# QuentinHuan/ENSEM3A_OpenCLRaytracer

Measured on AMD Instinct MI355X. Metric: Msamples/s Cornell box 1024x1024 64spp; 1/2/4/8-GPU scaling; HBM %peak, higher is better.
Workload: dtype f32; 1 GPU; cornell_1024_s64; scene=cornell, width=1024, height=1024, spp=64, max_bounce=4, traversal=fast, bvh=sah, parallelism=row-interleaved x1

## Files before the change

ensem3a_openclraytracer_amd/_native.py:

```python
from __future__ import annotations

import ctypes
import os
import threading

import numpy as np

from ._build import LIB

_lock = threading.Lock()
_lib = None
_host = None

RT_TRAVERSAL_FAST = 0
RT_TRAVERSAL_REF = 1
RT_BVH_REFERENCE = 0
RT_BVH_SAH = 1
RT_ERR_ARG = 1
RT_ERR_STATE = 3
RT_ACCUM_MAX_SAMPLES = 1 << 24

EXPORTED = (
    "rt_create", "rt_destroy", "rt_last_error", "rt_set_scene", "rt_set_env", "rt_set_option",
    "rt_render", "rt_render_device", "rt_tile_rows", "rt_count_work", "rt_count_work_detail", "rt_work_bytes", "rt_gamma",
    "rt_render_rgb8", "rt_rgb8_device", "rt_rgb8",
    "rt_accum_begin", "rt_accum_add", "rt_accum_add_rgb8", "rt_accum_read", "rt_accum_samples", "rt_accum_end",
    "rt_accum_begin_device", "rt_accum_add_device",
    "rt_accum_mark", "rt_accum_select", "rt_accum_select_mask", "rt_accum_select_all", "rt_accum_selection",
    "rt_accum_sample_map", "rt_accum_add_selected", "rt_accum_mark_device", "rt_accum_select_device",
    "rt_accum_select_mask_device", "rt_accum_select_all_device", "rt_accum_add_selected_device",
    "rt_accum_guides", "rt_accum_guides_device", "rt_denoise_device", "rt_accum_denoise",
    "rt_trace", "rt_trace_device",
    "rt_bvh_build", "rt_device_count", "rt_debug_math", "rt_debug_fn", "rt_debug_trace", "rt_debug_trace_clustered", "rt_debug_scene_info", "rt_debug_pixel_log",
    "rt_debug_wave_counts", "rt_debug_quantise_axis", "rt_debug_timings", "rt_debug_brute_layout",
    "rt_debug_brute_clusters", "rt_debug_brute_shell", "rt_debug_brute_near", "rt_debug_brute_quad",
    "rt_debug_brute_slices",
    "rt_debug_last_slices",
    "rt_debug_brute_refill", "rt_debug_last_refill", "rt_debug_last_launch",
    "rt_obj_parse", "rt_obj_size", "rt_obj_copy", "rt_obj_free", "rt_obj_last_error",
    "rt_scene_check", "rt_scene_last_error",
)
HOST_ONLY = ("rt_bvh_build", "rt_obj_parse", "rt_obj_size", "rt_obj_copy", "rt_obj_free", "rt_obj_last_error",
             "rt_scene_check", "rt_scene_last_error", "rt_debug_quantise_axis", "rt_debug_brute_layout",
             "rt_debug_brute_clusters", "rt_debug_brute_shell", "rt_debug_brute_near", "rt_debug_brute_quad")

_c_p = ctypes.c_void_p
_i64 = ctypes.c_int64
_i32 = ctypes.c_int


class DenoiseParams(ctypes.Structure):
    _fields_ = [("passes", ctypes.c_int), ("normal_squarings", ctypes.c_int),
                ("sigma_c", ctypes.c_float), ("sigma_p", ctypes.c_float)]

    def __init__(self, passes: int = 5, normal_squarings: int = 5, sigma_c: float = 1.5, sigma_p: float = 0.02):
        super().__init__(int(passes), int(normal_squarings), float(sigma_c), float(sigma_p))


GUIDE_FLOATS = 12

HIT_DTYPE = np.dtype([("k", np.float32), ("tri", np.int32), ("u", np.float32), ("v", np.float32)])
RAY_FLOATS = 8
RT_QUERY_CLOSEST = 0
RT_QUERY_ANY = 1
QUERY_HORIZON = 1000.0


def pack_rays(origins, directions, tmax=None) -> np.ndarray:
    o = np.asarray(origins, dtype=np.float32).reshape(-1, 3)
    d = np.asarray(directions, dtype=np.float32).reshape(-1, 3)
    if len(o) != len(d):
        raise ValueError(f"{len(o)} origins but {len(d)} directions")
    rays = np.zeros((len(o), RAY_FLOATS), np.float32)
    rays[:, 0:3] = d
    rays[:, 3:6] = o
    rays[:, 6] = QUERY_HORIZON if tmax is None else np.asarray(tmax, dtype=np.float32)
    return rays


class NativeError(RuntimeError):

    def __init__(self, status: int, message: str):
        super().__init__(f"[rt status {status}] {message}")
        self.status = status


def _preload_hip_runtime() -> None:
    import importlib.util
    try:
        spec = importlib.util.find_spec("torch")
    except (ImportError, ValueError):
        spec = None
    for d in (spec.submodule_search_locations or []) if spec else []:
        p = os.path.join(d, "lib", "libamdhip64.so")
        if os.path.exists(p):
            ctypes.CDLL(p, mode=ctypes.RTLD_GLOBAL)
            return


def lib():
    global _lib
    if _lib is not None:
        return _lib
    with _lock:
        if _lib is not None:
            return _lib
        _preload_hip_runtime()
        lib_path = os.environ.get("ENSEM3A_RT_LIB", LIB)
        if not os.path.exists(lib_path):
            raise RuntimeError(
                f"native library {lib_path} is missing: build it with "
                "`python -m ensem3a_openclraytracer_amd._build` (there is no CPU fallback)")
        L = ctypes.CDLL(lib_path)
        sig = {
            "rt_create": (_i32, [_i32, _c_p, ctypes.POINTER(_c_p)]),
            "rt_destroy": (None, [_c_p]),
            "rt_last_error": (ctypes.c_char_p, [_c_p]),
            "rt_set_scene": (_i32, [_c_p, _c_p, _i64, _c_p, _i64, _c_p, _i64, _c_p, _i64, _c_p, _i64, _c_p, _i64]),
# ... 342 lines not shown
        out = np.zeros((max(n, 1), GUIDE_FLOATS), np.float32)
        self._check(lib().rt_accum_guides(self.handle, out.ctypes.data))
        return out[:n]

    def accum_guides_device(self, d_guides_ptr: int, stream_ptr: int = 0, device_index: int = 0) -> None:
        self._check(lib().rt_accum_guides_device(self.handle, int(device_index),
                                                 _c_p(int(d_guides_ptr)) if d_guides_ptr else None,
                                                 self._stream(stream_ptr)))

    def denoise_device(self, d_rgb_ptr: int, d_guides_ptr: int, npix: int, width: int, d_out_ptr: int,
                       params: "DenoiseParams" = None, stream_ptr: int = 0, device_index: int = 0) -> None:
        self._check(lib().rt_denoise_device(self.handle, int(device_index),
                                            _c_p(int(d_rgb_ptr)) if d_rgb_ptr else None,
                                            _c_p(int(d_guides_ptr)) if d_guides_ptr else None, int(npix), int(width),
                                            ctypes.byref(params) if params is not None else None,
                                            _c_p(int(d_out_ptr)) if d_out_ptr else None, self._stream(stream_ptr)))

    def accum_denoise(self, params: "DenoiseParams" = None, out: np.ndarray = None) -> np.ndarray:
        out = self._accum_out(out, np.float32)
        self._check(lib().rt_accum_denoise(self.handle, ctypes.byref(params) if params is not None else None,
                                           out.ctypes.data))
        return out

    def trace(self, rays8, mode: int = RT_QUERY_CLOSEST) -> np.ndarray:
        r = f32(rays8)
        if r.size % RAY_FLOATS:
            raise ValueError("rays must hold 8 floats each: dir.xyz, origin.xyz, tmax, reserved")
        n = r.size // RAY_FLOATS
        out = np.zeros(n, HIT_DTYPE)
        self._check(lib().rt_trace(self.handle, ptr(r), n, int(mode), out.ctypes.data if n else None))
        return out

    def trace_device(self, device_index: int, rays_ptr: int, n: int, mode: int, out_ptr: int,
                     stream_ptr: int = 0) -> None:
        self._check(lib().rt_trace_device(self.handle, int(device_index), _c_p(int(rays_ptr)) if rays_ptr else None,
                                          int(n), int(mode), _c_p(int(out_ptr)) if out_ptr else None,
                                          self._stream(stream_ptr)))

    def rgb8(self, src, gamma: bool = False, out=None) -> np.ndarray:
        s = f32(src).reshape(-1)
        if out is None:
            out = np.zeros(s.size, dtype=np.uint8)
        self._check(lib().rt_rgb8(self.handle, ptr(s), out.ctypes.data, s.size, int(bool(gamma))))
        return out

    def rgb8_device(self, d_in_ptr: int, d_out_ptr: int, n: int, gamma: bool = False, stream_ptr: int = 0,
                    device_index: int = 0) -> None:
        self._check(lib().rt_rgb8_device(self.handle, int(device_index), _c_p(int(d_in_ptr)), _c_p(int(d_out_ptr)),
                                         int(n), int(bool(gamma)), _c_p(int(stream_ptr)) if stream_ptr else None))

    def debug_math(self, fn: int, x, y=None):
        x = f32(x)
        yy = f32(y) if y is not None else None
        out = np.zeros_like(x)
        self._check(lib().rt_debug_math(self.handle, int(fn), ptr(x), ptr(yy), out.ctypes.data, x.size))
        return out

    DEBUG_FN = {"camera": (0, 11, 3), "sun": (1, 5, 3), "hemi": (2, 6, 24), "ggx": (3, 13, 3), "ibl": (4, 4, 6),
                "mt_ref": (5, 24, 2), "mt_fast": (6, 24, 2), "box_ref": (7, 12, 1), "box_fast": (8, 13, 3)}

    def debug_fn(self, name: str, items) -> np.ndarray:
        fn, wi, wo = self.DEBUG_FN[name]
        x = f32(items)
        if x.ndim != 2 or x.shape[1] != wi:
            raise ValueError(f"{name}: items must be [n, {wi}] floats")
        out = np.zeros((x.shape[0], wo), dtype=np.float32)
        if x.shape[0]:
            self._check(lib().rt_debug_fn(self.handle, fn, ptr(x), out.ctypes.data, x.shape[0]))
        return out

    def debug_trace(self, rays, traversal: int):
        r = f32(rays).reshape(-1)
        out = np.zeros(2 * (r.size // 6), dtype=np.float32)
        self._check(lib().rt_debug_trace(self.handle, int(traversal), ptr(r), out.ctypes.data, r.size // 6))
        return out.reshape(-1, 2)

    def debug_trace_clustered(self, rays6):
        r = f32(rays6).reshape(-1, 6)
        out = np.zeros((len(r), 2), dtype=np.float32)
        info = np.zeros(4, dtype=np.int32)
        self._check(lib().rt_debug_trace_clustered(self.handle, r.ctypes.data, out.ctypes.data, len(r), info.ctypes.data))
        return out[:, 0].copy(), out[:, 1].copy().view(np.int32), info

    def debug_pixel_log(self, traversal, cam, env, npix, spp, max_bounce, pixel, cap=4096):
        c, e = f32(cam), f32(env)
        log = np.zeros((cap, 16), np.float32)
        n = ctypes.c_int(0)
        out3 = np.zeros(3, np.float32)
        self._check(lib().rt_debug_pixel_log(self.handle, int(traversal), ptr(c), ptr(e), int(npix), int(spp),
                                             int(max_bounce), int(pixel), log.ctypes.data, cap, ctypes.byref(n),
                                             out3.ctypes.data))
        return log[: n.value].copy(), out3

    def wave_counts(self, cam, env, npix, spp, max_bounce):
        c, e = f32(cam), f32(env)
        out = np.zeros(9, dtype=np.uint64)
        self._check(lib().rt_debug_wave_counts(self.handle, ptr(c), ptr(e), int(npix), int(spp), int(max_bounce),
                                               out.ctypes.data))
        keys = ("node_fetches", "tri_tests", "rays", "env_lookups", "stack_drops", "wave_trav_iters",
                "wave_render_iters", "cycles_shade", "cycles_trav")
        return {k: int(v) for k, v in zip(keys, out)}

    def scene_info(self):
        out = np.zeros(8, dtype=np.int64)
        self._check(lib().rt_debug_scene_info(self.handle, out.ctypes.data))
        return dict(fast_ok=bool(out[0]), depth=int(out[1]), nodes=int(out[2]), tris=int(out[3]),
                    brute_records=int(out[4]), brute_boxes=int(out[5]), wdq_omax=int(out[6]) * 1e-6)

    def timings(self) -> dict:
        out = np.zeros(4, dtype=np.float64)
        self._check(lib().rt_debug_timings(self.handle, out.ctypes.data))
        return dict(pack_ms=float(out[0]), upload_ms=float(out[1]), env_ms=float(out[2]), render_ms=float(out[3]))


def parse_obj(text):
    data = text.encode() if isinstance(text, str) else bytes(text)
    h = _c_p()
    H = host_lib()
    if H.rt_obj_parse(data, len(data), ctypes.byref(h)) != 0:
        raise ValueError("OBJ parse failed: " + H.rt_obj_last_error().decode(errors="replace"))
    try:
        n = [int(H.rt_obj_size(h, k)) for k in range(5)]
        vp, vn, vuv = (np.zeros(n[k], np.float32) for k in range(3))
        face = np.zeros(n[3], np.int32)
        H.rt_obj_copy(h, vp.ctypes.data, vn.ctypes.data, vuv.ctypes.data, face.ctypes.data)
    finally:
        H.rt_obj_free(h)
    return vp, vn, vuv, face, n[4]


def scene_check(V_p, V_n, faceData, materialData, bvh, layout: int = RT_BVH_SAH) -> dict:
    vp, vn, face, mat, b = f32(V_p), f32(V_n), i32(faceData), f32(materialData), f32(bvh)
    info = np.zeros(8, np.int64)
    H = host_lib()
    st = H.rt_scene_check(ptr(vp), vp.size, ptr(vn), vn.size, ptr(face), face.size, ptr(mat), mat.size,
                          ptr(b), b.size, int(layout), info.ctypes.data)
    msg = H.rt_scene_last_error().decode(errors="replace")
    if st != 0:
        raise NativeError(st, msg)
    return dict(tris=int(info[0]), nodes=int(info[1]), depth=int(info[2]), wnodes=int(info[3]),
                wdepth=int(info[4]), brute_records=int(info[5]), brute_boxes=int(info[6]), fast_ok=bool(info[7]),
                note=msg)


def brute_layout(V_p, V_n, faceData, materialData, bvh, layout: int = RT_BVH_SAH):
    vp, vn, face, mat, b = f32(V_p), f32(V_n), i32(faceData), f32(materialData), f32(bvh)
    H = host_lib()
    info = np.zeros(3, np.int64)
    args = (ptr(vp), vp.size, ptr(vn), vn.size, ptr(face), face.size, ptr(mat), mat.size, ptr(b), b.size, int(layout))
    st = H.rt_debug_brute_layout(*args, None, 0, info.ctypes.data)
    if st != 0:
        raise NativeError(st, H.rt_scene_last_error().decode(errors="replace"))
    boxes = np.zeros(int(info[2]), np.float32)
    st = H.rt_debug_brute_layout(*args, boxes.ctypes.data, boxes.size, info.ctypes.data)
    if st != 0:
        raise NativeError(st, H.rt_scene_last_error().decode(errors="replace"))
    return boxes.reshape(-1, 8), int(info[0]), int(info[1])


def brute_clusters(V_p, V_n, faceData, materialData, bvh, cluster: int = -1, layout: int = RT_BVH_SAH):
    vp, vn, face, mat, b = f32(V_p), f32(V_n), i32(faceData), f32(materialData), f32(bvh)
    H = host_lib()
    info = np.zeros(4, np.int64)
    args = (ptr(vp), vp.size, ptr(vn), vn.size, ptr(face), face.size, ptr(mat), mat.size, ptr(b), b.size, int(layout),
            int(cluster))
    st = H.rt_debug_brute_clusters(*args, None, 0, None, 0, info.ctypes.data)
    if st != 0:
        raise NativeError(st, H.rt_scene_last_error().decode(errors="replace"))
    slots, rows = np.zeros(int(info[2]), np.float32), np.zeros(int(info[3]), np.float32)
    st = H.rt_debug_brute_clusters(*args, slots.ctypes.data, slots.size, rows.ctypes.data, rows.size, info.ctypes.data)
    if st != 0:
        raise NativeError(st, H.rt_scene_last_error().decode(errors="replace"))
    return slots.reshape(-1, 8), rows.reshape(-1, 8), int(info[1])


SHELL_REC_FLOATS = 76


def brute_shell(V_p, V_n, faceData, materialData, bvh, cluster: int = -1, shell: int = -1, layout: int = RT_BVH_SAH):
    vp, vn, face, mat, b = f32(V_p), f32(V_n), i32(faceData), f32(materialData), f32(bvh)
    H = host_lib()
    info = np.zeros(3, np.int64)
    args = (ptr(vp), vp.size, ptr(vn), vn.size, ptr(face), face.size, ptr(mat), mat.size, ptr(b), b.size, int(layout),
            int(cluster), int(shell))
    st = H.rt_debug_brute_shell(*args, None, 0, info.ctypes.data)
    if st != 0:
        raise NativeError(st, H.rt_scene_last_error().decode(errors="replace"))
    if int(info[0]) == 0:
        return None
    rec = np.zeros(int(info[2]), np.float32)
    st = H.rt_debug_brute_shell(*args, rec.ctypes.data, rec.size, info.ctypes.data)
    if st != 0:
        raise NativeError(st, H.rt_scene_last_error().decode(errors="replace"))
    ints = rec[:SHELL_REC_FLOATS].view(np.int32)
    return dict(box=rec[:6].copy(), nrest=int(ints[6]), nfaces=int(ints[7]) & 0xff, faces=ints[8:20].reshape(6, 2).copy(),
                rest=rec[SHELL_REC_FLOATS:].reshape(-1, 8).copy())


NEAR_FLOOR = np.float32(0.0001) * (np.float32(1.0) - np.float32(2.0 ** -12))


def brute_near(V_p, V_n, faceData, materialData, bvh, cluster: int = -1, shell: int = -1, layout: int = RT_BVH_SAH):
    vp, vn, face, mat, b = f32(V_p), f32(V_n), i32(faceData), f32(materialData), f32(bvh)
    H = host_lib()
    info = np.zeros(2, np.int64)
    floor = np.zeros(1, np.float32)
    args = (ptr(vp), vp.size, ptr(vn), vn.size, ptr(face), face.size, ptr(mat), mat.size, ptr(b), b.size, int(layout),
            int(cluster), int(shell))
    st = H.rt_debug_brute_near(*args, None, 0, floor.ctypes.data, info.ctypes.data)
    if st != 0:
        raise NativeError(st, H.rt_scene_last_error().decode(errors="replace"))
    flags = np.zeros(int(info[0]), np.int32)
    st = H.rt_debug_brute_near(*args, flags.ctypes.data if flags.size else None, flags.size, floor.ctypes.data,
                               info.ctypes.data)
    if st != 0:
        raise NativeError(st, H.rt_scene_last_error().decode(errors="replace"))
    return flags.astype(bool), np.float32(floor[0]), int(info[1])


QUAD_BAND, QUAD_GRAZE, QUAD_DIR_MAX = np.float32(2.0 ** -8), np.float32(2.0 ** -6), np.float32(2.0)


def brute_quad(V_p, V_n, faceData, materialData, bvh, cluster: int = -1, shell: int = -1, quad: int = -1,
               layout: int = RT_BVH_SAH):
    vp, vn, face, mat, b = f32(V_p), f32(V_n), i32(faceData), f32(materialData), f32(bvh)
    flags, lines, words = np.zeros(6, np.int32), np.zeros(24, np.float32), np.zeros(18, np.int32)
    recs, guard, info = np.zeros(108, np.float32), np.zeros(3, np.float32), np.zeros(2, np.int64)
    st = host_lib().rt_debug_brute_quad(ptr(vp), vp.size, ptr(vn), vn.size, ptr(face), face.size, ptr(mat), mat.size,
                                        ptr(b), b.size, int(layout), int(cluster), int(shell), int(quad),
                                        flags.ctypes.data, lines.ctypes.data, words.ctypes.data, recs.ctypes.data,
                                        guard.ctypes.data,
                                        info.ctypes.data)
    if st != 0:
        raise NativeError(st, host_lib().rt_scene_last_error().decode(errors="replace"))
    return dict(split=(flags & 1).astype(bool), side=((flags >> 1) & 1).astype(bool), lines=lines.reshape(6, 4),
                words=words.view(np.uint32).reshape(6, 3), recs=recs.reshape(6, 2, 3, 3), guard=guard, nfaces=int(info[0]), nsplit=int(info[1]))


def brute_slices(nloc: int, lanes: int, spp: int, option: int = -1, accum_base: int = -1):
    out = np.zeros(3, np.int32)
    st = lib().rt_debug_brute_slices(int(nloc), int(lanes), int(spp), int(option), int(accum_base), out.ctypes.data)
    if st != 0:
        raise NativeError(st, "rt_debug_brute_slices: bad arguments")
    return bool(out[0]), int(out[1]), int(out[2])


def last_slices() -> int:
    return int(lib().rt_debug_last_slices())


def brute_refill(nloc: int, lanes: int, option: int = -1) -> int:
    out = np.zeros(1, np.int32)
    st = lib().rt_debug_brute_refill(int(nloc), int(lanes), int(option), out.ctypes.data)
    if st != 0:
        raise NativeError(st, "rt_debug_brute_refill: bad arguments")
    return int(out[0])


def last_refill():
    out = np.zeros(3, np.int64)
    st = lib().rt_debug_last_refill(out.ctypes.data)
    if st != 0:
        raise NativeError(st, "rt_debug_last_refill: bad arguments")
    return int(out[0]), int(out[1]), int(out[2])


LAUNCH_FIELDS = ("trav", "count", "log", "smem", "ovf", "resume", "step", "wide", "brute", "ts", "acc",
                 "team", "walk_team", "slices", "refill", "grid", "lds", "shell", "near", "quad")
BRUTE_SLICED = 4
BRUTE_REFILL = 8


def last_launch() -> dict:
    out = np.zeros(len(LAUNCH_FIELDS), np.int32)
    st = lib().rt_debug_last_launch(out.ctypes.data)
    if st != 0:
        raise NativeError(st, "rt_debug_last_launch: bad arguments")
    return {name: int(v) for name, v in zip(LAUNCH_FIELDS, out)}


def tile_rows(npix: int, width: int, row0: int, row_step: int) -> int:
    return int(lib().rt_tile_rows(int(npix), int(width), int(row0), int(row_step)))
```

ensem3a_openclraytracer_amd/csrc/rt_api.hip:

```cpp
#include <hip/hip_runtime.h>

#include <cmath>
#include <cstdarg>
#include <cstdio>
#include <algorithm>
#include <array>
#include <atomic>
#include <chrono>
#include <cstring>
#include <map>
#include <string>
#include <thread>
#include <vector>

#include "../../include/rt_api.h"
#include "../../include/rt_debug.h"
#include "rt_internal.h"
#include "scene_pack.h"

constexpr int kResumeMinBvh2 = 36, kResumeMinWide = 48;
constexpr int kDenoiseLds = 1;

using rt::HostScene;

namespace {

thread_local std::string g_thread_error;

struct DevBuf {
    void* p = nullptr;
    size_t bytes = 0;
    DevBuf() = default;
    DevBuf(const DevBuf&) = delete;
    DevBuf& operator=(const DevBuf&) = delete;
    DevBuf(DevBuf&& o) noexcept : p(o.p), bytes(o.bytes) { o.p = nullptr, o.bytes = 0; }
    DevBuf& operator=(DevBuf&& o) noexcept {
        std::swap(p, o.p);
        std::swap(bytes, o.bytes);
        return *this;
    }
    ~DevBuf() { release(); }
    void release() {
        if (p) (void)hipFree(p);
        p = nullptr;
        bytes = 0;
    }
};

struct Device {
    int id = 0;
    hipStream_t stream = nullptr;
    int cus = 0;
    DevBuf stack_ovf;
    DevBuf nodes, wnodes, wleaves, tri_fast, brute, brute_box, brute_cbox, brute_crow, bvh9, tri_geo, tri_shade, tri_frame, mat, ibl, ibl_sum, out, out8, counts, work, scratch_a, scratch_b;
    DevBuf pilot;
    DevBuf spec;
    DevBuf slice;
    DevBuf accum;
    bool acc_open = false;
    bool acc_valid = false;
    float acc_cam[10] = {0}, acc_env[5] = {0};
    int64_t acc_npix = 0, acc_nloc = 0, acc_samples = 0;
    int acc_max_bounce = 0, acc_row0 = 0, acc_row_step = 1;
    DevBuf mark, sel, all;
    bool acc_marked = false, acc_selected = false, acc_all_ready = false;
    bool acc_uniform = true;
    bool sel_all = false;
    int64_t sel_known = -1;
    int64_t acc_full = 0;
    DevBuf dn, dn_const, guides, dn_rgb, dn_guides, dn_out;
    DevBuf q_counter, q_rays, q_out;
    char* host_stage = nullptr;
    int* host_pick = nullptr;
    size_t host_stage_bytes = 0;
    hipEvent_t done = nullptr;
    hipStream_t last = nullptr;
    bool pending = false;

    Device() = default;
    Device(const Device&) = delete;
    Device& operator=(const Device&) = delete;
    ~Device() {
        (void)hipSetDevice(id);
        if (host_stage) (void)hipHostFree(host_stage);
        if (host_pick) (void)hipHostFree(host_pick);
        if (stream) (void)hipStreamDestroy(stream);
        if (done) (void)hipEventDestroy(done);
    }
};

}

struct rt_ctx {
    std::vector<Device> devs;
    HostScene hs;
    bool have_scene = false;
    bool have_env = false;
    int ibl_w = 0, ibl_h = 0;
    int traversal = RT_TRAVERSAL_FAST;
    int bvh_layout = RT_BVH_SAH;
    int brute_max = RT_BRUTE_MAX_DEFAULT;
    int brute_cluster = -1;
    int brute_shell = -1;
    int brute_near = -1;
    int brute_quad = -1;
    int resume_min = -1;
    int team = 0;
    int walk_team = 0;
    int max_waves = 0;
    int step = 0;
    int sun_skip = 1;
    int sun_any = 1;
    int block = 128;
    int bvh_width = 0;
    int fixed_point = 1;
    int sun_cache = 1;
    int pilot = -1;
    int pilot_chunk = 0;
    int pilot_levels = 0;
    int stack_lds = 0;
    int ref_stack = 20;
    int spec = -1;
    int wdq = 1;
    int handout = -1;
    int slices = -1;
    int brute_refill = -1;
    int denoise_lds = -1;
    int query_engine = 0;
    int query_grid = 0;
    bool accum_host = false;
    double t_pack_ms = 0, t_upload_ms = 0, t_env_ms = 0, t_render_ms = 0;
    std::string err;
};

namespace {

int set_err(rt_ctx* ctx, int code, const char* fmt, ...) {
    char buf[1024];
    va_list ap;
    va_start(ap, fmt);
    vsnprintf(buf, sizeof buf, fmt, ap);
    va_end(ap);
    if (ctx) ctx->err = buf;
    g_thread_error = buf;
    return code;
}

#define HIP_OR_RET(ctx, call)                                                                           \
    do {                                                                                                \
        hipError_t e_ = (call);                                                                         \
        if (e_ != hipSuccess)                                                                           \
            return set_err((ctx), RT_ERR_HIP, "%s failed: %s", #call, hipGetErrorString(e_));           \
    } while (0)

hipError_t grow(Device& d, DevBuf& b, size_t bytes) {
    bytes = std::max<size_t>(bytes, 16);
    if (b.p && b.bytes >= bytes) return hipSuccess;
    hipError_t e = d.pending ? hipEventSynchronize(d.done) : hipSuccess;
    if (e != hipSuccess) return e;
    if (b.p && (e = hipFree(b.p)) != hipSuccess) return e;
    b.p = nullptr;
    b.bytes = 0;
    if ((e = hipMalloc(&b.p, bytes)) == hipSuccess) b.bytes = bytes;
    return e;
}

hipError_t grow_stage(Device& d, size_t bytes) {
    if (d.host_stage_bytes >= bytes) return hipSuccess;
    hipError_t e = d.host_stage ? hipHostFree(d.host_stage) : hipSuccess;
    if (e != hipSuccess) return e;
    d.host_stage = nullptr;
    d.host_stage_bytes = 0;
    if ((e = hipHostMalloc((void**)&d.host_stage, bytes, hipHostMallocDefault)) == hipSuccess) d.host_stage_bytes = bytes;
    return e;
}

}

namespace {

constexpr int kStackLdsMin = 8;
hipError_t ensure_stack_ovf(Device& d, const HostScene& hs) {
    const int64_t extra = (int64_t)std::max(hs.depth, hs.wdepth) - kStackLdsMin;
    if (extra <= 0) return hipSuccess;
    return grow(d, d.stack_ovf, (size_t)std::max(d.cus, 1) * rt::kMaxLanesPerCu * (size_t)extra * sizeof(int2));
}

// ... 7 lines not shown
    d.pending = true;
    return hipEventRecord(d.done, s);
}

template <typename T>
hipError_t upload(Device& d, DevBuf& b, const std::vector<T>& v) {
    const size_t bytes = v.size() * sizeof(T);
    hipError_t e = grow(d, b, bytes);
    if (e != hipSuccess || bytes == 0) return e;
    return hipMemcpyAsync(b.p, v.data(), bytes, hipMemcpyHostToDevice, d.stream);
}

hipError_t upload_cbox(Device& d, const HostScene& hs) {
    if (hs.brute_shell.empty()) return upload(d, d.brute_cbox, hs.brute_cbox);
    std::vector<float> v(hs.brute_cbox);
    v.insert(v.end(), hs.brute_shell.begin(), hs.brute_shell.end());
    const hipError_t e = upload(d, d.brute_cbox, v);
    return e != hipSuccess ? e : hipStreamSynchronize(d.stream);
}

int upload_fast(rt_ctx* ctx, Device& d, const HostScene& hs) {
    HIP_OR_RET(ctx, hipSetDevice(d.id));
    HIP_OR_RET(ctx, order_after_last(d, d.stream));
    HIP_OR_RET(ctx, upload(d, d.nodes, hs.nodes));
    HIP_OR_RET(ctx, upload(d, d.wnodes, hs.wnodes));
    HIP_OR_RET(ctx, upload(d, d.wleaves, hs.wleaves));
    HIP_OR_RET(ctx, upload(d, d.brute, hs.brute));
    HIP_OR_RET(ctx, upload(d, d.brute_box, hs.brute_box));
    HIP_OR_RET(ctx, upload_cbox(d, hs));
    HIP_OR_RET(ctx, upload(d, d.brute_crow, hs.brute_crow));
    HIP_OR_RET(ctx, upload(d, d.tri_geo, hs.tri_geo));
    HIP_OR_RET(ctx, upload(d, d.tri_fast, hs.tri_fast));
    HIP_OR_RET(ctx, ensure_stack_ovf(d, hs));
    return RT_OK;
}

int effective_traversal(const rt_ctx* ctx) {
    return (ctx->traversal == RT_TRAVERSAL_FAST && ctx->hs.fast_ok) ? RT_TRAVERSAL_FAST : RT_TRAVERSAL_REF;
}

bool use_wide(const rt_ctx* ctx) {
    if (ctx->hs.wnodes.empty() || ctx->bvh_width == 2) return false;
    return ctx->bvh_width == 4 || (size_t)ctx->hs.nnodes * 16 * rt::kNodeF4 > rt::kWideMinBytes;
}

int resume_min_of(const rt_ctx* ctx) {
    return ctx->resume_min >= 0 ? ctx->resume_min : use_wide(ctx) ? kResumeMinWide : kResumeMinBvh2;
}

rt::DevScene dev_scene(const rt_ctx* ctx, const Device& d) {
    rt::DevScene s{};
    s.nodes = (const float4*)d.nodes.p;
    s.nnodes = ctx->hs.nnodes;
    s.root_ref = ctx->hs.root_ref;
    const bool wide = use_wide(ctx);
    s.wnodes = wide ? (const float4*)d.wnodes.p : nullptr;
    s.wleaves = wide ? (const float4*)d.wleaves.p : nullptr;
    s.wroot_ref = ctx->hs.wroot_ref;
    s.wdq_omax = wide ? ctx->hs.wdq_omax : 0.0f;
    for (int k = 0; k < 6; ++k) s.root_box[k] = ctx->hs.root_box[k];
    s.bvh9 = (const float*)d.bvh9.p;
    s.nbvh9 = ctx->hs.nbvh9;
    s.ref_stack = ctx->ref_stack;
    s.tri_geo = (const float4*)d.tri_geo.p;
    s.tri_fast = (const float4*)d.tri_fast.p;
    s.tri_shade = (const float4*)d.tri_shade.p;
    s.tri_frame = (const float4*)d.tri_frame.p;
    s.ntri = ctx->hs.ntri;
    s.mat = (const float*)d.mat.p;
    s.nmat = ctx->hs.nmat;
    s.ibl_sum = (const uint32_t*)d.ibl_sum.p;
    s.ibl_w = ctx->ibl_w;
    s.ibl_h = ctx->ibl_h;
    s.depth = wide ? std::max(ctx->hs.depth, ctx->hs.wdepth) : ctx->hs.depth;
    s.brute = (const float4*)d.brute.p;
    s.brute_box = (const float4*)d.brute_box.p;
    s.nbrute = ctx->hs.nbrute;
    s.nbox = ctx->hs.nbox;
    s.brute_cbox = (const float4*)d.brute_cbox.p;
    s.brute_crow = (const float4*)d.brute_crow.p;
    s.ncluster = ctx->hs.ncluster;
    s.ncslot = (int32_t)(ctx->hs.brute_cbox.size() / 8);
    s.nsingle4 = s.ncslot - rt::kClusterSlots * s.ncluster;
    s.host_flags = (ctx->brute_cluster < 0 ? rt::kHostClusterAuto : 0) | (ctx->hs.nquad > 0 ? rt::kHostQuad : 0);
    s.nsingle = ctx->hs.nsingle;
    s.shell = ctx->hs.nshell > 0 ? 2 * s.ncslot : 0;
    s.near_floor = s.shell && ctx->brute_near != 0 ? ctx->hs.shell_floor : 0.0f;
    s.near_mask_lo = s.near_floor != 0.0f ? (uint32_t)ctx->hs.shell_mask : 0u;
    s.near_mask_hi = s.near_floor != 0.0f ? (uint32_t)(ctx->hs.shell_mask >> 32) : 0u;
    s.stack_lds = std::min<int32_t>(s.depth > 0 ? s.depth : 1,
                                    ctx->stack_lds > 0 ? ctx->stack_lds : wide ? rt::kStackLdsWide : rt::kStackLds);
    s.stack_ovf = (int2*)d.stack_ovf.p;
    return s;
}

int check_frame(rt_ctx* ctx, const float* cam, const float* env, int64_t npix, int spp, int max_bounce, int row0,
                int row_step, rt::FrameParams* fp) {
    if (!ctx) return set_err(nullptr, RT_ERR_ARG, "null context");
    if (!ctx->have_scene) return set_err(ctx, RT_ERR_STATE, "rt_set_scene has not been called");
    if (!ctx->have_env) return set_err(ctx, RT_ERR_STATE, "rt_set_env has not been called");
    if (!cam || !env) return set_err(ctx, RT_ERR_ARG, "cam/env must not be NULL");
    if (!(cam[6] >= 1.0f) || !(cam[6] < 2147483648.0f))
        return set_err(ctx, RT_ERR_ARG, "cam[6] (row width) must be >= 1, got %g", (double)cam[6]);
    if (npix <= 0 || npix > 0x7fffffff) return set_err(ctx, RT_ERR_ARG, "pixel count %lld out of range", (long long)npix);
    if (spp < 0) return set_err(ctx, RT_ERR_ARG, "spp must be >= 0");
    if (row0 < 0 || row_step <= 0) return set_err(ctx, RT_ERR_ARG, "bad row tiling (%d, %d)", row0, row_step);
    if (max_bounce > 4096) return set_err(ctx, RT_ERR_ARG, "maxBounce %d > 4096", max_bounce);
    std::memcpy(fp->cam, cam, sizeof fp->cam);
    std::memcpy(fp->env, env, sizeof fp->env);
    fp->width = (int32_t)cam[6];
    fp->npix = npix;
    fp->spp = spp;
    fp->max_bounce = max_bounce;
    fp->row0 = row0;
    fp->row_step = row_step;
    fp->nloc = rt_tile_rows(npix, fp->width, row0, row_step) * fp->width;
    fp->log_pixel = -1;
    fp->resume_min = resume_min_of(ctx);
    fp->step = ctx->step;
    fp->sun_skip = (ctx->sun_skip && env[3] == 0.0f && env[4] >= 0.0f && ctx->hs.colors_finite) ? 1 : 0;
    fp->sun_any = (ctx->sun_any && !ctx->hs.has_glass) ? 1 : 0;
    fp->wide = use_wide(ctx) ? 1 : 0;
    fp->wdq = ctx->wdq;
    fp->fixed_point = ctx->fixed_point;
    fp->sun_cache = ctx->fixed_point && ctx->sun_cache ? 1 : 0;
    fp->pass = 0;
    fp->pilot = 0;
    fp->pilot_chunk = 1;
    fp->pilot_levels = 256;
    fp->pilot_state = nullptr;
    fp->pilot_draws = nullptr;
    fp->spec = 0;
    fp->spec_log = nullptr;
    fp->spec_cap = 0;
    fp->slices = 0;
    fp->refill = ctx->brute_refill;
    fp->slice_state = nullptr;
    fp->slice_ready = nullptr;
    fp->pilot_cost = nullptr;
    fp->pilot_order = nullptr;
    fp->team = ctx->team;
    fp->walk_team = ctx->walk_team;
    fp->max_waves = ctx->max_waves;
    fp->handout = ctx->handout >= 0 ? ctx->handout : (use_wide(ctx) && effective_traversal(ctx) == RT_TRAVERSAL_FAST);
    fp->log_buf = nullptr;
    fp->log_cap = 0;
    fp->log_count = nullptr;
    return RT_OK;
}

void invalidate_accum(rt_ctx* ctx) {
    for (auto& d : ctx->devs) {
        d.acc_valid = false;
        d.acc_marked = false;
        d.acc_selected = false;
    }
}

int slot_of(rt_ctx* ctx, int device_index, Device** d, const char* what = "device index") {
    if (!ctx) return set_err(nullptr, RT_ERR_ARG, "null context");
    if (device_index < 0 || device_index >= (int)ctx->devs.size())
        return set_err(ctx, RT_ERR_ARG, "%s %d out of range", what, device_index);
    *d = &ctx->devs[device_index];
    return RT_OK;
}

int repack_scene(rt_ctx* ctx) {
    if (!ctx->have_scene) return RT_OK;
    HostScene& hs = ctx->hs;
    std::string why;
    rt::pack_checked(hs, hs.bvh9.data(), hs.nbvh9, hs.ntri, ctx->bvh_layout, ctx->brute_max, ctx->brute_cluster,
                     ctx->brute_shell, ctx->brute_quad, why);
    for (auto& d : ctx->devs) {
        const int st = upload_fast(ctx, d, hs);
        if (st) return st;
        HIP_OR_RET(ctx, hipStreamSynchronize(d.stream));
    }
    if (!hs.fast_ok) ctx->err = "FAST traversal unavailable (" + why + "); REF traversal will be used";
    return RT_OK;
}

struct Accepts {
    enum Kind { kRange, kZeroOrRange, kSet } kind;
    int n;
    int64_t v[5];
    bool operator()(int64_t x) const {
        if (kind == kSet) return std::find(v, v + n, x) != v + n;
        return (kind == kZeroOrRange && x == 0) || (x >= v[0] && x <= v[1]);
    }
};
Accepts range(int64_t lo, int64_t hi) { return {Accepts::kRange, 2, {lo, hi}}; }
Accepts zero_or(int64_t lo, int64_t hi) { return {Accepts::kZeroOrRange, 2, {lo, hi}}; }
Accepts one_of(std::initializer_list<int64_t> members) {
    Accepts a{Accepts::kSet, (int)members.size(), {}};
    std::copy(members.begin(), members.end(), a.v);
    return a;
}

enum class Effect { kNone, kInvalidate, kRepack };

struct Option {
    const char* key;
    int rt_ctx::*field;
    Accepts accepts;
    std::string message;
    Effect effect;
};

std::string bounds_message(const char* fmt, int a, int b = 0) {
    char buf[128];
    snprintf(buf, sizeof buf, fmt, a, b);
    return buf;
}

const std::vector<Option>& options() {
    constexpr Effect none = Effect::kNone, invalidate = Effect::kInvalidate, repack = Effect::kRepack;
    static const std::vector<Option> table = {
        {"traversal", &rt_ctx::traversal, range(RT_TRAVERSAL_FAST, RT_TRAVERSAL_REF), "traversal must be 0 (fast) or 1 (ref)", invalidate},
        {"brute_near", &rt_ctx::brute_near, range(-1, 1), "brute_near must be -1 (auto), 0 (off) or 1 (auto)", none},
        {"brute_quad", &rt_ctx::brute_quad, range(-1, 1), "brute_quad must be -1 (auto), 0 (off) or 1 (auto)", repack},
        {"bvh", &rt_ctx::bvh_layout, range(RT_BVH_REFERENCE, RT_BVH_SAH), "bvh must be 0 (reference tree) or 1 (sah)", repack},
        {"brute_cluster", &rt_ctx::brute_cluster, range(-1, 1), "brute_cluster must be -1 (auto), 0 (off) or 1 (force)", repack},
        {"brute_shell", &rt_ctx::brute_shell, range(-1, 1), "brute_shell must be -1 (auto), 0 (off) or 1 (force)", repack},
        {"brute_max", &rt_ctx::brute_max, range(0, 4096), "brute_max must be in 0..4096", repack},
        {"resume_min", &rt_ctx::resume_min, range(-1, 64), "resume_min must be -1 (auto) or 0..64", none},
        {"team", &rt_ctx::team, one_of({0, 1, 2, 4, 8}), "team must be 0 (auto), 1, 2, 4 or 8", none},
        {"walk_team", &rt_ctx::walk_team, one_of({0, 1, 2, 4, 8}), "walk_team must be 0 (auto), 1, 2, 4 or 8", none},
        {"sun_any", &rt_ctx::sun_any, range(0, 1), "sun_any must be 0 or 1", none},
        {"sun_skip", &rt_ctx::sun_skip, range(0, 1), "sun_skip must be 0 or 1", none},
        {"step", &rt_ctx::step, range(0, 2), "step must be 0 (auto), 1 (item) or 2 (round)", none},
        {"waves", &rt_ctx::max_waves, range(0, 8), "waves must be in 0..8", none},
        {"pilot", &rt_ctx::pilot, range(-1, 1 << 20), "pilot must be -1 (auto), 0 (off) or a sample count", none},
        {"pilot_chunk", &rt_ctx::pilot_chunk, range(0, 4096), "pilot_chunk must be in 0..4096 (0 = auto)", none},
        {"pilot_levels", &rt_ctx::pilot_levels, zero_or(2, 256), "pilot_levels must be 0 (auto) or 2..256", none},
        {"stack_lds", &rt_ctx::stack_lds, zero_or(kStackLdsMin, rt::kStackLds),
         bounds_message("stack_lds must be 0 (auto) or %d..%d", kStackLdsMin, rt::kStackLds), none},
        {"sun_cache", &rt_ctx::sun_cache, range(0, 1), "sun_cache must be 0 or 1", none},
        {"fixed_point", &rt_ctx::fixed_point, range(0, 1), "fixed_point must be 0 or 1", none},
        {"bvh_width", &rt_ctx::bvh_width, one_of({0, 2, 4}), "bvh_width must be 0 (auto), 2 or 4", none},
        {"ref_stack", &rt_ctx::ref_stack, range(20, 64), "ref_stack must be in 20..64 (20 = the reference's)", invalidate},
        {"slices", &rt_ctx::slices, range(-1, 16), "slices must be -1 (auto), 0 (off) or 1..16", none},
        {"brute_refill", &rt_ctx::brute_refill, range(-1, rt::kRefillMax),
         bounds_message("brute_refill must be -1 (auto), 0 or 1 (off) or 2..%d", rt::kRefillMax), none},
        {"denoise_lds", &rt_ctx::denoise_lds, range(-1, 1), "denoise_lds must be -1 (auto), 0 or 1", none},
        {"query_engine", &rt_ctx::query_engine, range(0, 2), "query_engine must be 0 (auto), 1 (plain) or 2 (persistent)", none},
        {"query_grid", &rt_ctx::query_grid, range(0, 1 << 20), "query_grid must be 0 (auto) or a block count", none},
        {"wdq", &rt_ctx::wdq, range(0, 1), "wdq must be 0 or 1", none},
        {"handout", &rt_ctx::handout, range(-1, 1), "handout must be -1 (auto), 0 or 1", none},
        {"spec", &rt_ctx::spec, one_of({-1, 0, 2, 4, 8}), "spec must be -1 (auto), 0 (off), 2, 4 or 8", none},
        {"block", &rt_ctx::block, one_of({64, 128, 256}), "block must be 64/128/256", none},
    };
    return table;
}

}

extern "C" {

int rt_device_count(void) {
    int n = 0;
    if (hipGetDeviceCount(&n) != hipSuccess) return 0;
    return n;
}

int rt_create(int n_devices, const int* device_ids, rt_ctx** out) {
    if (!out) return set_err(nullptr, RT_ERR_ARG, "out must not be NULL");
    *out = nullptr;
    int avail = 0;
    hipError_t e = hipGetDeviceCount(&avail);
    if (e != hipSuccess || avail <= 0)
        return set_err(nullptr, RT_ERR_HIP, "no HIP device available (%s)", hipGetErrorString(e));
    if (n_devices <= 0) n_devices = 1;
    if (!device_ids && n_devices > avail)
        return set_err(nullptr, RT_ERR_ARG, "requested %d devices, %d available", n_devices, avail);
    if (n_devices > 64) return set_err(nullptr, RT_ERR_ARG, "at most 64 device slots, got %d", n_devices);
    rt_ctx* ctx = new rt_ctx();
    ctx->devs = std::vector<Device>(n_devices);
    for (int i = 0; i < n_devices; ++i) {
        const int id = device_ids ? device_ids[i] : i;
        if (id < 0 || id >= avail) {
            delete ctx;
            return set_err(nullptr, RT_ERR_ARG, "device id %d out of range", id);
        }
        ctx->devs[i].id = id;
        if ((e = hipSetDevice(id)) != hipSuccess ||
            (e = hipStreamCreateWithFlags(&ctx->devs[i].stream, hipStreamNonBlocking)) != hipSuccess ||
            (e = hipEventCreateWithFlags(&ctx->devs[i].done, hipEventDisableTiming)) != hipSuccess ||
            (e = hipDeviceGetAttribute(&ctx->devs[i].cus, hipDeviceAttributeMultiprocessorCount, id)) != hipSuccess) {
            rt_destroy(ctx);
            return set_err(nullptr, RT_ERR_HIP, "device %d init failed: %s", id, hipGetErrorString(e));
        }
    }
    *out = ctx;
    return RT_OK;
}

void rt_destroy(rt_ctx* ctx) {
    if (!ctx) return;
    for (auto& d : ctx->devs) {
        if (hipSetDevice(d.id) != hipSuccess) continue;
        if (d.pending) (void)hipEventSynchronize(d.done);
        if (d.stream) (void)hipStreamSynchronize(d.stream);
    }
    delete ctx;
}

const char* rt_last_error(rt_ctx* ctx) { return ctx ? ctx->err.c_str() : g_thread_error.c_str(); }

int rt_set_option(rt_ctx* ctx, const char* key, int64_t value) {
    if (!ctx || !key) return set_err(ctx, RT_ERR_ARG, "null argument");
    for (const Option& o : options()) {
        if (std::strcmp(key, o.key)) continue;
        if (!o.accepts(value)) return set_err(ctx, RT_ERR_ARG, "%s", o.message.c_str());
        ctx->*o.field = (int)value;
        if (o.effect == Effect::kInvalidate) invalidate_accum(ctx);
        return o.effect == Effect::kRepack ? repack_scene(ctx) : RT_OK;
    }
    return set_err(ctx, RT_ERR_ARG, "unknown option '%s'", key);
}

int rt_set_scene(rt_ctx* ctx, const float* vp, int64_t nvp, const float* vn, int64_t nvn, const float* vuv,
                 int64_t nvuv, const int32_t* face, int64_t nface, const float* mat, int64_t nmat, const float* bvh9,
                 int64_t nbvh) {
    (void)vuv;
    (void)nvuv;
    if (!ctx) return set_err(nullptr, RT_ERR_ARG, "null context");
    const auto t0 = std::chrono::steady_clock::now();
    HostScene hs;
    std::string msg, why;
    const int rc = rt::scene_prepare(hs, vp, nvp, vn, nvn, face, nface, mat, nmat, bvh9, nbvh, ctx->bvh_layout,
                                     ctx->brute_max, ctx->brute_cluster, ctx->brute_shell, ctx->brute_quad, msg, why);
    if (rc != RT_OK) return set_err(ctx, rc, "%s", msg.c_str());
    invalidate_accum(ctx);
    const auto t1 = std::chrono::steady_clock::now();
    for (auto& d : ctx->devs) {
        const int st = upload_fast(ctx, d, hs);
        if (st) return st;
        HIP_OR_RET(ctx, upload(d, d.bvh9, hs.bvh9));
        HIP_OR_RET(ctx, upload(d, d.tri_shade, hs.tri_shade));
        HIP_OR_RET(ctx, upload(d, d.mat, hs.mat));
        HIP_OR_RET(ctx, grow(d, d.tri_frame, (size_t)std::max<int64_t>(hs.ntri, 1) * 3 * sizeof(float4)));
        HIP_OR_RET(ctx, grow(d, d.work, rt::kWorkBytes));
        HIP_OR_RET(ctx, hipStreamSynchronize(d.stream));
    }
    ctx->hs = std::move(hs);
    for (auto& d : ctx->devs) {
        HIP_OR_RET(ctx, hipSetDevice(d.id));
        HIP_OR_RET(ctx, rt::launch_prep_frames(dev_scene(ctx, d), (float4*)d.tri_frame.p, d.stream));
        HIP_OR_RET(ctx, hipStreamSynchronize(d.stream));
    }
    ctx->have_scene = true;
    ctx->t_pack_ms = std::chrono::duration<double, std::milli>(t1 - t0).count();
    ctx->t_upload_ms = std::chrono::duration<double, std::milli>(std::chrono::steady_clock::now() - t1).count();
    if (!ctx->hs.fast_ok) ctx->err = "FAST traversal unavailable (" + why + "); REF traversal will be used";
    return RT_OK;
}

int rt_set_env(rt_ctx* ctx, const uint8_t* rgba, int w, int h) {
    if (!ctx) return set_err(nullptr, RT_ERR_ARG, "null context");
    if (!rgba || w <= 0 || h <= 0) return set_err(ctx, RT_ERR_ARG, "bad IBL image (%d x %d)", w, h);
    const size_t bytes = (size_t)w * h * 4;
    invalidate_accum(ctx);
    const auto t0 = std::chrono::steady_clock::now();
    for (auto& d : ctx->devs) {
        HIP_OR_RET(ctx, hipSetDevice(d.id));
        HIP_OR_RET(ctx, order_after_last(d, d.stream));
        HIP_OR_RET(ctx, grow(d, d.ibl, bytes));
        HIP_OR_RET(ctx, grow(d, d.ibl_sum, (size_t)(w + 1) * (size_t)(h + 1) * sizeof(uint32_t)));
        HIP_OR_RET(ctx, hipMemcpyAsync(d.ibl.p, rgba, bytes, hipMemcpyHostToDevice, d.stream));
        HIP_OR_RET(ctx, rt::launch_ibl_sum((const uchar4*)d.ibl.p, w, h, (uint32_t*)d.ibl_sum.p, d.stream));
        HIP_OR_RET(ctx, hipStreamSynchronize(d.stream));
    }
    ctx->ibl_w = w;
    ctx->ibl_h = h;
    ctx->have_env = true;
    ctx->t_env_ms = std::chrono::duration<double, std::milli>(std::chrono::steady_clock::now() - t0).count();
    return RT_OK;
}

int64_t rt_tile_rows(int64_t npix, int width, int row0, int row_step) {
    if (npix <= 0 || width <= 0 || row0 < 0 || row_step <= 0) return 0;
    const int64_t H = (npix + width - 1) / width;
    if (row0 >= H) return 0;
    return (H - row0 + row_step - 1) / row_step;
}

namespace {
constexpr int kSlicesWide = 8;
constexpr int kSlicesWideSmall = 12;
constexpr int64_t kSlicesMinPerLane = 4;
using rt::kAccumSliceMin;

hipError_t setup_pilot(rt_ctx* ctx, Device& d, rt::FrameParams& fp) {
    if (ctx->pilot == 0 || effective_traversal(ctx) != RT_TRAVERSAL_FAST || fp.nloc <= 0 || use_wide(ctx))
        return hipSuccess;
    int k = ctx->pilot;
    if (k < 0) {
        const int64_t lanes = (int64_t)std::max(d.cus, 1) * rt::kWalkLanesPerCu;
        if (ctx->hs.nbrute > 0 || use_wide(ctx) || fp.spp < 16 || fp.nloc > 16 * lanes) return hipSuccess;
        if (ctx->slices != 0 && fp.nloc >= kSlicesMinPerLane * lanes) return hipSuccess;
        k = fp.spp / 8;
    }
    if (k >= fp.spp) return hipSuccess;
    const size_t n = (size_t)fp.nloc;
    const size_t need = n * 40 + 2 * 256 * sizeof(uint32_t) + 2 * (n + 1) * sizeof(uint32_t) +
                        (n + 256) * sizeof(uint32_t) + n * sizeof(uint32_t);
    hipError_t e = grow(d, d.pilot, need);
    if (e != hipSuccess) return e;
    char* base = (char*)d.pilot.p;
    fp.pilot = k;
    fp.pilot_chunk = ctx->pilot_chunk > 0 ? ctx->pilot_chunk : (ctx->hs.nbrute > 0 ? 64 : 1);
    fp.pilot_levels = ctx->pilot_levels > 0 ? ctx->pilot_levels : 256;
    fp.pilot_state = (float4*)base;
    fp.pilot_cost = (uint32_t*)(base + n * 32);
    fp.pilot_order = (const uint32_t*)(base + n * 36);
// ... 991 lines not shown
        return set_err(ctx, RT_ERR_STATE, "FAST traversal unavailable for this scene");
    if (!n) return RT_OK;
    Device& d = ctx->devs[0];
    HIP_OR_RET(ctx, hipSetDevice(d.id));
    HIP_OR_RET(ctx, grow(d, d.scratch_a, (size_t)n * 6 * sizeof(float)));
    HIP_OR_RET(ctx, grow(d, d.scratch_b, (size_t)n * 2 * sizeof(float)));
    HIP_OR_RET(ctx, hipMemcpyAsync(d.scratch_a.p, rays, (size_t)n * 6 * sizeof(float), hipMemcpyHostToDevice, d.stream));
    HIP_OR_RET(ctx, order_after_last(d, d.stream));
    HIP_OR_RET(ctx, rt::launch_debug_trace(dev_scene(ctx, d), traversal, (const float*)d.scratch_a.p,
                                           (float*)d.scratch_b.p, n, d.stream));
    HIP_OR_RET(ctx, hipMemcpyAsync(out, d.scratch_b.p, (size_t)n * 2 * sizeof(float), hipMemcpyDeviceToHost, d.stream));
    HIP_OR_RET(ctx, hipStreamSynchronize(d.stream));
    return RT_OK;
}

int rt_debug_trace_clustered(rt_ctx* ctx, const float* rays, float* out, int64_t n, int32_t info[4]) {
    if (!ctx || !rays || !out || !info || n < 0) return set_err(ctx, RT_ERR_ARG, "bad arguments");
    if (!ctx->have_scene) return set_err(ctx, RT_ERR_STATE, "no scene");
    if (ctx->hs.nbrute <= 0 || ctx->hs.ncluster <= 0)
        return set_err(ctx, RT_ERR_ARG, "the scene has no clustered brute-force array (%d records, %d clusters; option "
                       "\"brute_cluster\" %d)", (int)ctx->hs.nbrute, (int)ctx->hs.ncluster, ctx->brute_cluster);
    Device& d = ctx->devs[0];
    HIP_OR_RET(ctx, hipSetDevice(d.id));
    HIP_OR_RET(ctx, grow(d, d.scratch_a, (size_t)n * 6 * sizeof(float)));
    HIP_OR_RET(ctx, grow(d, d.scratch_b, (size_t)n * 2 * sizeof(float)));
    if (n) HIP_OR_RET(ctx, hipMemcpyAsync(d.scratch_a.p, rays, (size_t)n * 6 * sizeof(float), hipMemcpyHostToDevice, d.stream));
    HIP_OR_RET(ctx, order_after_last(d, d.stream));
    HIP_OR_RET(ctx, rt::launch_debug_trace_clustered(dev_scene(ctx, d), (const float*)d.scratch_a.p,
                                                     (float*)d.scratch_b.p, n, info, d.stream));
    if (n) HIP_OR_RET(ctx, hipMemcpyAsync(out, d.scratch_b.p, (size_t)n * 2 * sizeof(float), hipMemcpyDeviceToHost, d.stream));
    HIP_OR_RET(ctx, hipStreamSynchronize(d.stream));
    return RT_OK;
}

int rt_debug_pixel_log(rt_ctx* ctx, int traversal, const float cam[10], const float env[5], int64_t npix, int spp,
                       int max_bounce, int64_t pixel, float* log, int cap, int* n_events, float out3[3]) {
    rt::FrameParams fp;
    if (!cam) return set_err(ctx, RT_ERR_ARG, "null cam");
    const int W = (int)cam[6];
    if (W <= 0 || pixel < 0 || pixel >= npix) return set_err(ctx, RT_ERR_ARG, "pixel out of range");
    int st = check_frame(ctx, cam, env, npix, spp, 0, (int)(pixel / W), (int)npix, &fp);
    if (st) return st;
    if (!log || cap <= 0 || !n_events || !out3) return set_err(ctx, RT_ERR_ARG, "bad log buffer");
    if (traversal == RT_TRAVERSAL_FAST && !ctx->hs.fast_ok) traversal = RT_TRAVERSAL_REF;
    fp.max_bounce = max_bounce;
    fp.sun_skip = 0;
    fp.sun_any = 0;
    Device& d = ctx->devs[0];
    HIP_OR_RET(ctx, hipSetDevice(d.id));
    const size_t obytes = (size_t)fp.nloc * 3 * sizeof(float);
    const size_t lbytes = (size_t)cap * 16 * sizeof(float);
    HIP_OR_RET(ctx, grow(d, d.scratch_a, obytes + lbytes + 16));
    float* dout = (float*)d.scratch_a.p;
    fp.log_buf = dout + fp.nloc * 3;
    fp.log_count = (int32_t*)(fp.log_buf + (size_t)cap * 16);
    fp.log_cap = cap;
    fp.log_pixel = pixel;
    HIP_OR_RET(ctx, hipMemsetAsync(fp.log_count, 0, sizeof(int32_t), d.stream));
    HIP_OR_RET(ctx, order_after_last(d, d.stream));
    HIP_OR_RET(ctx, rt::launch_debug_log(dev_scene(ctx, d), fp, traversal, dout, (unsigned int*)d.work.p, d.stream));
    HIP_OR_RET(ctx, mark_launch(d, d.stream));
    int32_t n = 0;
    HIP_OR_RET(ctx, hipMemcpyAsync(&n, fp.log_count, sizeof n, hipMemcpyDeviceToHost, d.stream));
    HIP_OR_RET(ctx, hipStreamSynchronize(d.stream));
    if (n > cap) n = cap;
    HIP_OR_RET(ctx, hipMemcpy(log, fp.log_buf, (size_t)n * 16 * sizeof(float), hipMemcpyDeviceToHost));
    HIP_OR_RET(ctx, hipMemcpy(out3, dout + 3 * (pixel % W), 3 * sizeof(float), hipMemcpyDeviceToHost));
    *n_events = n;
    return RT_OK;
}

int rt_debug_brute_slices(int64_t nloc, int64_t lanes, int spp, int option, int accum_base, int32_t out[3]) {
    if (!out || nloc < 0 || lanes < 0 || option < -1 || option > 16) return RT_ERR_ARG;
    const int todo = spp - std::max(accum_base, 0);
    const int v = rt::brute_slice_launch(rt::brute_slice_offer(option, todo, accum_base >= 0), nloc, lanes);
    out[0] = v != 0;
    out[1] = v & 0xff;
    out[2] = v >> 8;
    return RT_OK;
}

int rt_debug_last_slices(void) { return rt::last_launch().slices; }

int rt_debug_last_launch(int32_t out[20]) {
    if (!out) return RT_ERR_ARG;
    const rt::LaunchNote n = rt::last_launch();
    const rt::KernelKey& k = n.key;
    const int64_t v[20] = {k.trav, k.count, k.log,  k.smem,       k.ovf,    k.resume, k.step, k.wide,          k.brute,
                           k.ts,   k.acc,   n.team, n.walk_team,  n.slices, n.refill, n.grid, (int64_t)n.lds,
                           n.shell, n.near, n.quad};
    for (int i = 0; i < 20; ++i) out[i] = (int32_t)std::min<int64_t>(v[i], INT32_MAX);
    return RT_OK;
}

int rt_debug_brute_refill(int64_t nloc, int64_t lanes, int option, int32_t* out) {
    if (!out || nloc < 0 || lanes < 0 || option < -1 || option > rt::kRefillMax) return RT_ERR_ARG;
    *out = rt::brute_refill_launch(option, nloc, lanes);
    return RT_OK;
}

int rt_debug_last_refill(int64_t out[3]) {
    if (!out) return RT_ERR_ARG;
    out[0] = rt::last_launch().refill;
    out[1] = g_refill_events.load(std::memory_order_relaxed);
    out[2] = g_refill_lanes.load(std::memory_order_relaxed);
    return RT_OK;
}

int rt_debug_timings(rt_ctx* ctx, double out[4]) {
    if (!ctx || !out) return set_err(ctx, RT_ERR_ARG, "bad arguments");
    out[0] = ctx->t_pack_ms;
    out[1] = ctx->t_upload_ms;
    out[2] = ctx->t_env_ms;
    out[3] = ctx->t_render_ms;
    return RT_OK;
}

int rt_debug_scene_info(rt_ctx* ctx, int64_t out[8]) {
    if (!ctx || !out) return set_err(ctx, RT_ERR_ARG, "bad arguments");
    out[0] = ctx->hs.fast_ok ? 1 : 0;
    out[1] = ctx->hs.depth;
    out[2] = ctx->hs.nnodes;
    out[3] = ctx->hs.ntri;
    out[4] = effective_traversal(ctx) == RT_TRAVERSAL_FAST ? ctx->hs.nbrute : 0;
    out[5] = out[4] ? ctx->hs.nbox : 0;
    out[6] = ctx->hs.wnodes.empty() ? 0 : (int64_t)std::llround((double)ctx->hs.wdq_omax * 1e6);
    out[7] = 0;
    return RT_OK;
}

}
```

ensem3a_openclraytracer_amd/csrc/rt_debug_fn.hip:

```cpp
#include "../../include/rt_debug.h"
#include "rt_device.h"

namespace rt {

namespace {

static_assert(RT_FN_COUNT == kDebugFns, "debug_fn_in / debug_fn_out list every function");

__device__ __forceinline__ float ubits(uint32_t u) { return __uint_as_float(u); }
__device__ __forceinline__ rtm_f3 ld3(const float* p) { return rtm_v3(p[0], p[1], p[2]); }
__device__ __forceinline__ void st3(float* p, rtm_f3 v) { p[0] = v.x; p[1] = v.y; p[2] = v.z; }

__global__ void debug_camera_kernel(const float* __restrict__ in, float* __restrict__ out, int64_t n) {
    const int64_t i = (int64_t)blockIdx.x * blockDim.x + threadIdx.x;
    if (i >= n) return;
    const float* x = in + debug_fn_in(RT_FN_CAMERA) * i;
    FrameParams F{};
    for (int k = 0; k < 10; ++k) F.cam[k] = x[k];
    F.width = (int)x[6];
    const LaunchConst C = make_const(F);
    st3(out + 3 * i, camera_dir(C, F.width, __float_as_int(x[10])));
}

__global__ void debug_sun_kernel(const float* __restrict__ in, float* __restrict__ out, int64_t n) {
// ... 17 lines not shown
}

__global__ void debug_hemi_kernel(const float* __restrict__ in, const float4* __restrict__ tri_shade,
                                  const float4* __restrict__ frame, float* __restrict__ out, int64_t n) {
    const int64_t i = (int64_t)blockIdx.x * blockDim.x + threadIdx.x;
    if (i >= n) return;
    const float* x = in + debug_fn_in(RT_FN_HEMI) * i;
    const rtm_f3 nrm = xyz(tri_shade[i]);
    const float4 f0 = frame[3 * i], f1 = frame[3 * i + 1], f2 = frame[3 * i + 2];
    float* o = out + debug_fn_out(RT_FN_HEMI) * i;
    for (int form = 0; form < 4; ++form) {
        uint32_t s0 = __float_as_uint(x[4]), s1 = __float_as_uint(x[5]);
        float inv = 0.0f;
        rtm_f3 d;
        if (form == 0) d = hemi_cosine(nrm, f0, f1, f2, &s0, &s1, &inv);
        else if (form == 1) d = hemi_uniform(nrm, f0, f1, f2, &s0, &s1, &inv);
        else d = hemi_sample(form == 2, nrm, f0, f1, f2, &s0, &s1, &inv);
        st3(o + 6 * form, d);
        o[6 * form + 3] = inv;
        o[6 * form + 4] = ubits(s0);
        o[6 * form + 5] = ubits(s1);
    }
}

__global__ void debug_ggx_kernel(const float* __restrict__ in, float* __restrict__ out, int64_t n) {
    const int64_t i = (int64_t)blockIdx.x * blockDim.x + threadIdx.x;
    if (i >= n) return;
    const float* x = in + debug_fn_in(RT_FN_GGX) * i;
    st3(out + 3 * i, brdf_ggx(ld3(x), x[3], ld3(x + 4), ld3(x + 7), ld3(x + 10)));
}

__global__ void debug_ibl_kernel(DevScene S, const float* __restrict__ in, float* __restrict__ out, int64_t n) {
    const int64_t i = (int64_t)blockIdx.x * blockDim.x + threadIdx.x;
    if (i >= n) return;
    const float* x = in + debug_fn_in(RT_FN_IBL) * i;
    FrameParams F{};
    F.cam[6] = 1.0f;
    F.cam[9] = 1.0f;
    const LaunchConst C = make_const(F);
    Cnt c{};
    st3(out + 6 * i, sample_ibl<false>(S, C, ld3(x), c));
    st3(out + 6 * i + 3, sample_ibl_if<false>(S, C, ld3(x), x[3], c));
}

template <bool FAST>
__global__ void debug_mt_kernel(const float* __restrict__ in, float* __restrict__ out, int64_t n) {
    const int64_t i = (int64_t)blockIdx.x * blockDim.x + threadIdx.x;
    if (i >= n) return;
    static_assert(debug_fn_in(RT_FN_MT_REF) == 24 && debug_fn_in(RT_FN_MT_FAST) == 24, "six float4 per item");
    const float4* rec = reinterpret_cast<const float4*>(in) + 6 * i;
    const float* r = in + 24 * i + 12;
    const rtm_f3 d = ld3(r), o = ld3(r + 3);
    float k = 1000.0f;
    int rank = 0;
    bool hit;
    if (FAST) hit = mt_core(xyz(rec[0]), xyz(rec[1]), xyz(rec[2]), o, d, &k);
    else hit = mt_test(rec, 0, o, d, &k, &rank);
    out[2 * i] = hit ? 1.0f : 0.0f;
    out[2 * i + 1] = k;
}

__global__ void debug_box_ref_kernel(const float* __restrict__ in, float* __restrict__ out, int64_t n) {
    const int64_t i = (int64_t)blockIdx.x * blockDim.x + threadIdx.x;
    if (i >= n) return;
    const float* x = in + debug_fn_in(RT_FN_BOX_REF) * i;
    out[i] = ref_box(x + 6, ld3(x + 3), ld3(x)) ? 1.0f : 0.0f;
}

__global__ void debug_box_fast_kernel(const float* __restrict__ in, float* __restrict__ out, int64_t n) {
    const int64_t i = (int64_t)blockIdx.x * blockDim.x + threadIdx.x;
    if (i >= n) return;
    const float* x = in + debug_fn_in(RT_FN_BOX_FAST) * i;
    const rtm_f3 d = ld3(x), o = ld3(x + 3);
    const float ix = dev_recip(d.x), iy = dev_recip(d.y), iz = dev_recip(d.z);
    float tmin, tmax;
    slab(x[6], x[9], x[7], x[10], x[8], x[11], o, ix, iy, iz, tmin, tmax);
    out[3 * i] = box_hit(tmin, tmax, x[12]) ? 1.0f : 0.0f;
    out[3 * i + 1] = tmin;
    out[3 * i + 2] = tmax;
}

__global__ void __launch_bounds__(256) debug_trace_clustered_kernel(DevScene S, const float* __restrict__ rays,
                                                                    float* __restrict__ out, int64_t n) {
    extern __shared__ int lds_stack[];
    const int B = blockDim.x;
    float4* lr = reinterpret_cast<float4*>(reinterpret_cast<char*>(lds_stack) + (B / 64) * BRUTE_WAVE_LDS);
    float4* lc = lr + 3 * S.nbrute;
    for (int q = threadIdx.x; q < 3 * S.nbrute; q += B) lr[q] = S.brute[4 * (q / 3) + 1 + q % 3];
    for (int q = threadIdx.x; q < 2 * S.ncslot; q += B) lc[q] = S.brute_cbox[q];
    if (S.shell)
        for (int q = threadIdx.x; q < 2 * kShellRows; q += B) lc[S.shell + q] = S.brute_cbox[S.shell + kShellRowF4 + q];
    __syncthreads();
    const int64_t i = (int64_t)blockIdx.x * B + threadIdx.x;
    if (i >= n) return;
    const float* r = rays + 6 * i;
    Cnt c{};
    const Hit h = trace_brute_compact<false, true>(S, ld3(r + 3), ld3(r), reinterpret_cast<char*>(lds_stack) +
                                                                          (threadIdx.x >> 6) * BRUTE_WAVE_LDS,
                                                   lr, 3u, c, 1, lc);
    out[2 * i] = h.k;
    out[2 * i + 1] = __int_as_float(h.tri);
}

}

static size_t debug_clustered_lds_bytes(const DevScene& sc, int block) {
    return (size_t)(block / 64) * BRUTE_WAVE_LDS + (size_t)sc.nbrute * 48 + (size_t)sc.ncslot * 32 +
           (sc.shell ? (size_t)kShellRows * 32 : 0);
}

hipError_t launch_debug_trace_clustered(const DevScene& sc, const float* rays, float* out, int64_t n, int32_t info[4],
                                        hipStream_t stream) {
    const int block = 256;
    const size_t lds = debug_clustered_lds_bytes(sc, block);
    if (sc.nbrute <= 0 || sc.ncluster <= 0 || lds > 64 * 1024 || n > (int64_t)INT_MAX * block) return hipErrorInvalidValue;
    const int shell = sc.shell != 0;
    info[0] = sc.ncluster;
    info[1] = shell;
    info[2] = shell && sc.near_floor != 0.0f;
    info[3] = shell && (sc.host_flags & kHostQuad) != 0;
    if (n <= 0) return hipSuccess;
    hipLaunchKernelGGL(debug_trace_clustered_kernel, dim3((unsigned)((n + block - 1) / block)), dim3(block), lds, stream,
                       sc, rays, out, n);
    return hipGetLastError();
}

size_t debug_fn_scratch_bytes(int fn, int64_t n) {
    return fn == RT_FN_HEMI ? (size_t)n * 4 * sizeof(float4) + 2 * kMatF * sizeof(float) : 0;
}

hipError_t launch_debug_fn(const DevScene& sc, int fn, const float* in, float* out, int64_t n, void* scratch,
                           hipStream_t stream) {
    if (n <= 0) return hipSuccess;
    const dim3 block(256), grid((unsigned)((n + 255) / 256));
    switch (fn) {
        case RT_FN_CAMERA: hipLaunchKernelGGL(debug_camera_kernel, grid, block, 0, stream, in, out, n); break;
        case RT_FN_SUN: hipLaunchKernelGGL(debug_sun_kernel, grid, block, 0, stream, in, out, n); break;
        case RT_FN_HEMI: {
            if (n > INT_MAX) return hipErrorInvalidValue;
            float4* shade = static_cast<float4*>(scratch);
            float4* frame = shade + n;
            float* mat = reinterpret_cast<float*>(frame + 3 * n);
            hipLaunchKernelGGL(debug_hemi_scene_kernel, grid, block, 0, stream, in, shade, mat, n);
            hipLaunchKernelGGL(prep_frames_kernel, grid, block, 0, stream, (const float4*)shade, (const float*)mat,
                               (int)n, frame);
            hipLaunchKernelGGL(debug_hemi_kernel, grid, block, 0, stream, in, (const float4*)shade,
                               (const float4*)frame, out, n);
            break;
        }
        case RT_FN_GGX: hipLaunchKernelGGL(debug_ggx_kernel, grid, block, 0, stream, in, out, n); break;
        case RT_FN_IBL:
            if (!sc.ibl_sum || sc.ibl_w <= 0 || sc.ibl_h <= 0) return hipErrorInvalidValue;
            hipLaunchKernelGGL(debug_ibl_kernel, grid, block, 0, stream, sc, in, out, n);
            break;
        case RT_FN_MT_REF: hipLaunchKernelGGL(debug_mt_kernel<false>, grid, block, 0, stream, in, out, n); break;
        case RT_FN_MT_FAST: hipLaunchKernelGGL(debug_mt_kernel<true>, grid, block, 0, stream, in, out, n); break;
        case RT_FN_BOX_REF: hipLaunchKernelGGL(debug_box_ref_kernel, grid, block, 0, stream, in, out, n); break;
        case RT_FN_BOX_FAST: hipLaunchKernelGGL(debug_box_fast_kernel, grid, block, 0, stream, in, out, n); break;
        default: return hipErrorInvalidValue;
    }
    return hipGetLastError();
}

}
```

ensem3a_openclraytracer_amd/csrc/rt_device.h:

```cpp
#pragma once
#include <algorithm>
#include <climits>

#include "rt_internal.h"
#include "rtm.h"

namespace rt {

namespace {

constexpr size_t kLdsSceneMax = 24 * 1024;

constexpr int TRAV_FAST = 0;
constexpr int TRAV_REF = 1;
constexpr int REF_STACK = 20;

struct Hit {
    float k;
    int tri;
};

struct Cnt {
    unsigned long long nodes, tris, rays, env, dropped;
    unsigned long long wave_trav;
// ... 301 lines not shown
        }
        if (item == 0x7fffffff) break;
    }
    if (best.tri >= 0) best.tri = (int)((unsigned)best.tri / 48u);
    return best;
}

typedef const float __attribute__((address_space(4))) const_f;
struct ConstF4 {
    const const_f* p;
    __device__ __forceinline__ float4 operator[](int i) const {
        return make_float4(p[4 * i], p[4 * i + 1], p[4 * i + 2], p[4 * i + 3]);
    }
};
__device__ __forceinline__ ConstF4 as_const(const float4* p) {
    return ConstF4{(const const_f*)(const float*)(p)};
}

__device__ __forceinline__ float sgpr1(float x) {
    return __int_as_float(__builtin_amdgcn_readfirstlane(__float_as_int(x)));
}
__device__ __forceinline__ float4 sgpr4(float4 v) {
    return make_float4(sgpr1(v.x), sgpr1(v.y), sgpr1(v.z), sgpr1(v.w));
}

constexpr unsigned BRUTE_RING = 256u;
constexpr unsigned BRUTE_OWNERS = 128u;
constexpr int BRUTE_INV_OFF = 64 * 6 * 4 + 64 * 8 + (BRUTE_RING + 64) * 4;
#ifndef RT_CHAIN_STAMPS
#define RT_CHAIN_STAMPS 0
#endif
#ifndef RT_SHADE_ROWS
#define RT_SHADE_ROWS 1
#endif
constexpr int BRUTE_STAMP_OFF = BRUTE_INV_OFF + 64 * 3 * 4 + BRUTE_OWNERS * 4;
constexpr int BRUTE_WAVE_LDS = BRUTE_STAMP_OFF + (RT_CHAIN_STAMPS ? 64 : 0);
enum { kStampHead = 0, kStampShell, kStampSingles, kStampClusters, kStampBatches, kStampTail, kStampRest, kStampN };
__device__ __forceinline__ void chain_stamp(char* wl, int done) {
#if RT_CHAIN_STAMPS
    const unsigned long long act = __ballot(1);
    if ((threadIdx.x & 63) == (unsigned)__ffsll((long long)act) - 1u) {
        unsigned long long* st = reinterpret_cast<unsigned long long*>(wl + BRUTE_STAMP_OFF);
        const unsigned long long now = clock64();
        st[done] += now - st[kStampN];
        st[kStampN] = now;
    }
#endif
}
static_assert(kClusterLockNum >= 0 && kClusterLockNum <= 8 && BRUTE_OWNERS >= 64 + 64 / kClusterSlots + 2, "owner list");

__device__ __forceinline__ unsigned lane_prefix(unsigned long long m, unsigned base) {
    return __builtin_amdgcn_mbcnt_hi((unsigned)(m >> 32), __builtin_amdgcn_mbcnt_lo((unsigned)m, base));
}

__device__ __forceinline__ void wave_lds_sync() {
    __builtin_amdgcn_fence(__ATOMIC_SEQ_CST, "wavefront");
    __builtin_amdgcn_wave_barrier();
}

__device__ __forceinline__ float near_floor_of(const DevScene& S, int g) {
    const uint32_t m = g < 32 ? S.near_mask_lo : S.near_mask_hi;
    return g < 64 && ((m >> (g & 31)) & 1u) ? kNearFloor : 0.0f;
}

__device__ __forceinline__ float max3_f32(float a, float b, float c) {
    float r;
    asm("v_max3_f32 %0, %1, %2, %3" : "=v"(r) : "v"(a), "v"(b), "v"(c));
    return r;
}
__device__ __forceinline__ float min3_f32(float a, float b, float c) {
    float r;
    asm("v_min3_f32 %0, %1, %2, %3" : "=v"(r) : "v"(a), "v"(b), "v"(c));
    return r;
}

__device__ __forceinline__ unsigned quad_pick(float4 ln, float4 wd, rtm_f3 o, rtm_f3 d, float tin, float T, float da) {
    const float sg = fmaf(ln.x, fmaf(T, d.x, o.x), fmaf(ln.y, fmaf(T, d.y, o.y), fmaf(ln.z, fmaf(T, d.z, o.z), ln.w)));
    const float dm = fmaxf(fmaxf(fabsf(d.x), fabsf(d.y)), fabsf(d.z));
    const bool sure = (tin <= 0.0f) & (T >= 0.0f) & (fabsf(da) >= kQuadGraze * dm) & (dm <= kQuadDirMax) &
                      (fabsf(sg) >= kQuadBand);
    return __float_as_uint(sure ? (sg >= 0.0f ? wd.y : wd.z) : wd.x);
}

template <int N> struct IntC { static constexpr int value = N; };
static_assert(kBoxGroup == 1 || kBoxGroup == 2 || kBoxGroup == 4 || kBoxGroup == 8, "the lock-step tail is cut into powers of two");

template <bool COUNT, bool CLU = false>
__device__ Hit trace_brute_compact(const DevScene& S, rtm_f3 o, rtm_f3 d, char* wl, const float4* mtrec,
                                   unsigned mtstride, Cnt& c, int ts = 1, const float4* boxrec = nullptr) {
    const unsigned lane = threadIdx.x & 63;
    const unsigned sub = lane & (unsigned)(ts - 1), tl = lane - sub;
    if (COUNT && sub == 0) c.rays++;
    const unsigned long long act = __ballot(1);
    const int nact = __popcll(act);
    const int myrank = (int)lane_prefix(act, 0u);
    float* ray = reinterpret_cast<float*>(wl);
    unsigned long long* bestk = reinterpret_cast<unsigned long long*>(wl + 64 * 6 * 4);
    unsigned* ring = reinterpret_cast<unsigned*>(wl + 64 * 6 * 4 + 64 * 8);
    ray[0 * 64 + lane] = o.x; ray[1 * 64 + lane] = o.y; ray[2 * 64 + lane] = o.z;
    ray[3 * 64 + lane] = d.x; ray[4 * 64 + lane] = d.y; ray[5 * 64 + lane] = d.z;
    const unsigned long long nokey = ((unsigned long long)__float_as_uint(1000.0f) << 32) | 0xffffffffull;
    bestk[lane] = nokey;
    wave_lds_sync();
    const float ix = dev_recip(d.x), iy = dev_recip(d.y), iz = dev_recip(d.z);
    float bk = 1000.0f;
    unsigned head = 0, tail = 0;
    [[maybe_unused]] int sec = kStampShell;
    auto run_batch = [&](int n) __attribute__((always_inline)) {
        if constexpr (CLU && !COUNT) chain_stamp(wl, sec);
        if (myrank < n) {
            const unsigned e = ring[(head + myrank) & (BRUTE_RING - 1)];
            const unsigned ow = e >> 16, q = e & 0xffffu;
            const rtm_f3 ro = rtm_v3(ray[ow], ray[64 + ow], ray[128 + ow]);
            const rtm_f3 rd = rtm_v3(ray[192 + ow], ray[256 + ow], ray[320 + ow]);
            const float4* rq = mtrec + mtstride * q;
            const float4 r1 = rq[0], r2 = rq[1], r3 = rq[2];
            const rtm_f3 a = rtm_v3(r1.z, r1.w, r2.x), e1 = rtm_v3(r2.y, r2.z, r2.w), e2 = rtm_v3(r3.x, r3.y, r3.z);
            const rtm_f3 h = rtm_cross(rd, e2);
            const float det = rtm_dot(e1, h);
            const float f = mt_recip(det);
            const rtm_f3 sv = rtm_sub(ro, a);
            const float u = f * rtm_dot(sv, h);
            const rtm_f3 qv = rtm_cross(sv, e1);
            const float v = f * rtm_dot(rd, qv);
            const float k = f * rtm_dot(e2, qv);
            const bool parallel = det > -0.0000001f && det < 0.0000001f;
            const bool hit = !parallel && !(u < 0.0f || u > 1.0f) && !(v < 0.0f || u + v > 1.0f) &&
                             (k > 0.0000001f) && k > 0.0001f && k < 1000.0f;
            if (hit) atomicMin(&bestk[ow], ((unsigned long long)__float_as_uint(k) << 32) | q);
        }
        head += n;
        wave_lds_sync();
        if constexpr (CLU && !COUNT) chain_stamp(wl, kStampBatches);
    };
    auto enqueue = [&](bool pass, unsigned qa, int qb) __attribute__((always_inline)) {
        const unsigned long long m = __ballot(pass);
        if (m == 0) return;
        const unsigned n = (unsigned)__popcll(m);
        if (COUNT && pass) c.tris += qb >= 0 ? 2 : 1;
        const unsigned r = lane_prefix(m, tail);
        ring[pass ? (r & (BRUTE_RING - 1)) : BRUTE_RING + lane] = (tl << 16) | qa;
        if (qb >= 0) ring[pass ? ((r + n) & (BRUTE_RING - 1)) : BRUTE_RING + lane] = (tl << 16) | (unsigned)qb;
        tail += qb >= 0 ? 2 * n : n;
        wave_lds_sync();
        if ((int)(tail - head) >= nact) {
            do run_batch(nact); while ((int)(tail - head) >= nact);
            bk = __uint_as_float((unsigned)(bestk[tl] >> 32));
        }
    };
    unsigned cq_pk = 0;
    auto group = [&](auto wc, const ConstF4 cb, int g0, int nreal) __attribute__((always_inline)) {
        constexpr int W = decltype(wc)::value;
        float4 bx[2 * W];
#pragma unroll
        for (int j = 0; j < 2 * W; ++j) bx[j] = sgpr4(cb[2 * g0 + j]);
        const float cull = bk * CULL_MARGIN;
        bool pass[W];
#pragma unroll
        for (int j = 0; j < W; ++j) {
            float tn, tx;
            slab(bx[2 * j].x, bx[2 * j].y, bx[2 * j].z, bx[2 * j].w, bx[2 * j + 1].x, bx[2 * j + 1].y, o, ix, iy, iz,
                 tn, tx);
            if constexpr (COUNT && !CLU) pass[j] = fmaxf(tn, near_floor_of(S, g0 + j)) <= fminf(tx, cull);
            else pass[j] = box_hit(tn, tx, cull);
        }
#pragma unroll
        for (int j = 0; j < W; ++j) {
            if (COUNT && g0 + j >= nreal) break;
            const int qa = __float_as_int(bx[2 * j + 1].z), qb = __float_as_int(bx[2 * j + 1].w);
            if (COUNT) {
                c.boxes++;
                count_wave(c.wave_trav); c.nodes++;
                if (qb >= 0) { count_wave(c.wave_trav); c.nodes++; }
            }
            if constexpr (COUNT && !CLU) {
                const unsigned keep = cq_pk & 0xffffu;
                const bool one = pass[j] && qb >= 0 && cq_pk >= 0xffff0000u && (keep == (unsigned)qa || keep == (unsigned)qb);
                enqueue(pass[j] && !one, (unsigned)qa, qb);
                enqueue(one, keep, -1);
            } else {
                enqueue(pass[j], (unsigned)qa, qb);
            }
        }
    };
    auto lockstep_padded = [&](const ConstF4 cb, int gb, int ge) __attribute__((always_inline)) {
        for (int g0 = gb; g0 < ge; g0 += kBoxGroup) group(IntC<kBoxGroup>{}, cb, g0, ge);
    };
    auto lockstep = [&](const ConstF4 cb, int gb, int ge) __attribute__((always_inline)) {
        int g0 = gb;
        for (; g0 + kBoxGroup <= ge; g0 += kBoxGroup) group(IntC<kBoxGroup>{}, cb, g0, ge);
        const int rem = ge - g0;
        if constexpr (kBoxGroup > 4) if (rem & 4) group(IntC<4>{}, cb, g0 + (rem & ~7), ge);
        if constexpr (kBoxGroup > 2) if (rem & 2) group(IntC<2>{}, cb, g0 + (rem & ~3), ge);
        if constexpr (kBoxGroup > 1) if (rem & 1) group(IntC<1>{}, cb, g0 + (rem & ~1), ge);
    };
    if (CLU) {
        float* inv = reinterpret_cast<float*>(wl + BRUTE_INV_OFF);
        unsigned* olist = reinterpret_cast<unsigned*>(wl + BRUTE_INV_OFF + 64 * 3 * 4);
        const unsigned* besthi = reinterpret_cast<const unsigned*>(bestk) + 1;
        inv[lane] = ix; inv[64 + lane] = iy; inv[128 + lane] = iz;
        const ConstF4 cb = as_const(S.brute_cbox);
        ConstF4 sb = cb;
        int ns = S.nsingle;
        if (S.shell) {
            const ConstF4 sh{cb.p + 4 * S.shell};
            const float4 h0 = sgpr4(sh[0]), h1 = sgpr4(sh[1]), fx = sgpr4(sh[2]), fy = sgpr4(sh[3]), fz = sgpr4(sh[4]);
            const int nquad = __float_as_int(h1.w) >> 8;
            const float cull = bk * CULL_MARGIN, nearf = S.near_floor;
            const float x0 = (h0.x - o.x) * ix, x1 = (h0.y - o.x) * ix;
            const float y0 = (h0.z - o.y) * iy, y1 = (h0.w - o.y) * iy;
            const float z0 = (h1.x - o.z) * iz, z1 = (h1.y - o.z) * iz;
            const float t[6] = {x0, x1, y0, y1, z0, z1};
            const float mn[3] = {fminf(x0, x1), fminf(y0, y1), fminf(z0, z1)};
            const float mx[3] = {fmaxf(x0, x1), fmaxf(y0, y1), fmaxf(z0, z1)};
            const int q[12] = {__float_as_int(fx.x), __float_as_int(fx.y), __float_as_int(fx.z), __float_as_int(fx.w),
                               __float_as_int(fy.x), __float_as_int(fy.y), __float_as_int(fy.z), __float_as_int(fy.w),
                               __float_as_int(fz.x), __float_as_int(fz.y), __float_as_int(fz.z), __float_as_int(fz.w)};
            bool pass[6];
#pragma unroll
            for (int f = 0; f < 6; ++f) {
                const int a = f >> 1;
                const float tn = fmaxf(fmaxf(a == 0 ? t[f] : mn[0], a == 1 ? t[f] : mn[1]), a == 2 ? t[f] : mn[2]);
                const float tx = fminf(fminf(a == 0 ? t[f] : mx[0], a == 1 ? t[f] : mx[1]), a == 2 ? t[f] : mx[2]);
                pass[f] = fmaxf(tn, nearf) <= fminf(tx, cull);
            }
            unsigned long long many = 0;
            int npass = 0;
#pragma unroll
            for (int f = 0; f < 6; ++f) {
                const unsigned long long mf = __ballot(pass[f]);
                many |= mf;
                npass += __popcll(mf);
            }
            if (npass == __popcll(many)) {
                int row = 2 * 6;
#pragma unroll
                for (int f = 0; f < 6; ++f) row = pass[f] ? 2 * f : row;
                const float4* rw = boxrec + S.shell + row;
                unsigned pk;
                if (nquad) {
                    const float da = (pass[0] || pass[1]) ? d.x : (pass[2] || pass[3]) ? d.y : d.z;
                    pk = quad_pick(rw[0], rw[1], o, d, max3_f32(mn[0], mn[1], mn[2]), min3_f32(mx[0], mx[1], mx[2]), da);
                } else {
                    pk = __float_as_uint(rw[1].x);
                }
                const bool p1 = pk != ~0u, p2 = pk < 0xffff0000u;
                const unsigned long long m1 = __ballot(p1);
                if (m1 != 0) {
                    const unsigned long long m2 = __ballot(p2);
                    const unsigned n1 = (unsigned)__popcll(m1);
                    if (COUNT && p1) c.tris += p2 ? 2 : 1;
                    const unsigned r1 = lane_prefix(m1, tail), r2 = lane_prefix(m2, tail + n1);
                    ring[p1 ? (r1 & (BRUTE_RING - 1)) : BRUTE_RING + lane] = (tl << 16) | (pk & 0xffffu);
                    ring[p2 ? (r2 & (BRUTE_RING - 1)) : BRUTE_RING + lane] = (tl << 16) | (pk >> 16);
                    tail += n1 + (unsigned)__popcll(m2);
                    wave_lds_sync();
                    if ((int)(tail - head) >= nact) {
                        do run_batch(nact); while ((int)(tail - head) >= nact);
                        bk = __uint_as_float((unsigned)(bestk[tl] >> 32));
                    }
                }
            } else {
#pragma unroll
                for (int f = 0; f < 6; ++f)
                    if (q[2 * f] >= 0) enqueue(pass[f], (unsigned)q[2 * f], q[2 * f + 1]);
            }
            sb = ConstF4{sh.p + kShellRecF};
            ns = __float_as_int(h1.z);
        }
        if constexpr (!COUNT) { chain_stamp(wl, kStampShell); sec = kStampSingles; }
        lockstep(sb, 0, ns);
        if constexpr (!COUNT) { chain_stamp(wl, kStampSingles); sec = kStampClusters; }
        unsigned ihead = 0, itail = 0;
        auto run_items = [&](int n) __attribute__((always_inline)) {
            bool pass = false;
            unsigned ow = 0, qa = 0;
            int qb = -1;
            if (myrank < n) {
                const unsigned i = ihead + (unsigned)myrank;
                const unsigned e = olist[(i >> kClusterShift) & (BRUTE_OWNERS - 1)];
                ow = e & 63u;
                const unsigned slot = (e >> 8) + (i & (unsigned)(kClusterSlots - 1));
                const rtm_f3 ro = rtm_v3(ray[ow], ray[64 + ow], ray[128 + ow]);
                const float4 b0 = boxrec[2 * slot], b1 = boxrec[2 * slot + 1];
                float tn, tx;
                slab(b0.x, b0.y, b0.z, b0.w, b1.x, b1.y, ro, inv[ow], inv[64 + ow], inv[128 + ow], tn, tx);
                pass = box_hit(tn, tx, __uint_as_float(besthi[2 * ow]) * CULL_MARGIN);
                qa = (unsigned)__float_as_int(b1.z);
                qb = __float_as_int(b1.w);
            }
            ihead += (unsigned)n;
            const bool pass2 = pass && qb >= 0;
            const unsigned long long m = __ballot(pass), m2 = __ballot(pass2);
            if (m == 0) return;
            const unsigned np = (unsigned)__popcll(m);
            if (pass) ring[lane_prefix(m, tail) & (BRUTE_RING - 1)] = (ow << 16) | qa;
            if (pass2) ring[lane_prefix(m2, tail + np) & (BRUTE_RING - 1)] = (ow << 16) | (unsigned)qb;
            tail += np + (unsigned)__popcll(m2);
            wave_lds_sync();
            if ((int)(tail - head) >= nact) {
                do run_batch(nact); while ((int)(tail - head) >= nact);
                bk = __uint_as_float((unsigned)(bestk[tl] >> 32));
            }
        };
        const ConstF4 cr = as_const(S.brute_crow);
        const int lock = (nact * kClusterLockNum) >> 3;
        for (int cl = 0; cl < S.ncluster; ++cl) {
            const float4 u0 = sgpr4(cr[2 * cl]), u1 = sgpr4(cr[2 * cl + 1]);
            float tn, tx;
            slab(u0.x, u0.y, u0.z, u0.w, u1.x, u1.y, o, ix, iy, iz, tn, tx);
            const bool pass = box_hit(tn, tx, bk * CULL_MARGIN);
            const unsigned long long m = __ballot(pass);
            if (m == 0) continue;
            const int np = __popcll(m);
            const int first = __float_as_int(u1.z);
            if (np > lock) {
                lockstep(cb, first, first + __float_as_int(u1.w));
                continue;
            }
            if (pass) olist[lane_prefix(m, itail >> kClusterShift) & (BRUTE_OWNERS - 1)] = lane | ((unsigned)first << 8);
            itail += (unsigned)np << kClusterShift;
            wave_lds_sync();
            while ((int)(itail - ihead) >= nact) run_items(nact);
        }
        while (itail != ihead) run_items(min((int)(itail - ihead), nact));
        if constexpr (!COUNT) { chain_stamp(wl, kStampClusters); sec = kStampTail; }
    } else if (ts == 1) {
        if constexpr (COUNT) {
            if (S.shell) {
                const ConstF4 sh{as_const(S.brute_cbox).p + 4 * S.shell};
                const float4 h0 = sgpr4(sh[0]), h1 = sgpr4(sh[1]);
                const float cull = bk * CULL_MARGIN, nearf = S.near_floor;
                const float x0 = (h0.x - o.x) * ix, x1 = (h0.y - o.x) * ix;
                const float y0 = (h0.z - o.y) * iy, y1 = (h0.w - o.y) * iy;
                const float z0 = (h1.x - o.z) * iz, z1 = (h1.y - o.z) * iz;
                const float t[6] = {x0, x1, y0, y1, z0, z1};
                const float mn[3] = {fminf(x0, x1), fminf(y0, y1), fminf(z0, z1)};
                const float mx[3] = {fmaxf(x0, x1), fmaxf(y0, y1), fmaxf(z0, z1)};
                unsigned long long many = 0;
                int npass = 0, row = 2 * 6;
                bool pass[6];
                for (int f = 0; f < 6; ++f) {
                    const int a = f >> 1;
                    const float tn = fmaxf(fmaxf(a == 0 ? t[f] : mn[0], a == 1 ? t[f] : mn[1]), a == 2 ? t[f] : mn[2]);
                    const float tx = fminf(fminf(a == 0 ? t[f] : mx[0], a == 1 ? t[f] : mx[1]), a == 2 ? t[f] : mx[2]);
                    pass[f] = fmaxf(tn, nearf) <= fminf(tx, cull);
                    const unsigned long long mf = __ballot(pass[f]);
                    many |= mf;
                    npass += __popcll(mf);
                    row = pass[f] ? 2 * f : row;
                }
                if (npass == __popcll(many)) {
                    const float4* rw = S.brute_cbox + S.shell + kShellRowF4 + row;
                    const float da = (pass[0] || pass[1]) ? d.x : (pass[2] || pass[3]) ? d.y : d.z;
                    cq_pk = quad_pick(rw[0], rw[1], o, d, max3_f32(mn[0], mn[1], mn[2]), min3_f32(mx[0], mx[1], mx[2]), da);
                }
            }
        }
        lockstep_padded(as_const(S.brute_box), 0, S.nbox);
    } else {
        const int rounds = (S.nbox + ts - 1) / ts;
        for (int gg = 0; gg < rounds; ++gg) {
            if (COUNT) { count_wave(c.wave_trav); count_wave(c.wave_trav); }
            const int g = gg * ts + (int)sub;
            bool pass = false;
            int qa = 0, qb = -1;
            if (g < S.nbox) {
                const float4 b0 = boxrec[2 * g], b1 = boxrec[2 * g + 1];
                float tn, tx;
                slab(b0.x, b0.y, b0.z, b0.w, b1.x, b1.y, o, ix, iy, iz, tn, tx);
                if constexpr (COUNT) pass = fmaxf(tn, near_floor_of(S, g)) <= fminf(tx, bk * CULL_MARGIN);
                else pass = box_hit(tn, tx, bk * CULL_MARGIN);
                qa = __float_as_int(b1.z);
                qb = __float_as_int(b1.w);
                if (COUNT) { c.nodes += qb >= 0 ? 2 : 1; c.boxes++; }
            }
            enqueue(pass, (unsigned)qa, -1);
            enqueue(pass && qb >= 0, (unsigned)qb, -1);
        }
    }
    while (tail != head) run_batch(min((int)(tail - head), nact));
    const unsigned long long key = bestk[tl];
    Hit best{1000.0f, -1};
    if (key != nokey) {
        best.k = __uint_as_float((unsigned)(key >> 32));
        best.tri = __float_as_int(mtrec[mtstride * (unsigned)(key & 0xffffffffu) + 2].w);
    }
    if constexpr (CLU && !COUNT) chain_stamp(wl, kStampTail);
    return best;
}

template <int TRAV, bool COUNT, bool SOA = false, bool OVF = false, bool BLDS = false, bool CLU = false>
__device__ __forceinline__ Hit trace(const DevScene& S, const float4* nodes, const float4* tris, rtm_f3 o, rtm_f3 d,
                                     int* stk, int B, const LaneStack& st, Cnt& c, const float4* mtrec = nullptr,
                                     int ts = 1, const float4* boxrec = nullptr) {
    if (TRAV == TRAV_REF) return trace_ref<COUNT>(S, o, d, stk, B, c);
    if (S.nbrute > 0)
        return trace_brute_compact<COUNT, CLU>(S, o, d, reinterpret_cast<char*>(stk - threadIdx.x) +
                                                        (threadIdx.x >> 6) * BRUTE_WAVE_LDS,
                                          BLDS ? mtrec : S.brute + 1, BLDS ? 3u : 4u, c, BLDS ? ts : 1, boxrec);
    return trace_fast<COUNT, SOA, OVF>(S, nodes, tris, o, d, st, c);
}

struct LaunchConst {
    rtm_rot cam_rx, cam_ry, cam_rz;
    rtm_rot ibl_x, ibl_y;
    rtm_f3 focal, position, sun;
    float pas;
};

__host__ __device__ inline LaunchConst make_const(const FrameParams& F) {
    LaunchConst c;
    const float* cam = F.cam;
    c.focal = rtm_v3(cam[0], cam[1] - (1.0f / (2.0f * rtm_tan(cam[9] / 2.0f))), cam[2]);
    c.position = rtm_v3(cam[0], cam[1], cam[2]);
    c.pas = 1.0f / cam[6];
    c.cam_rx = rtm_rot_prepare(cam[3] * (3.14f / 180.0f), rtm_v3(1, 0, 0));
    c.cam_ry = rtm_rot_prepare(cam[4] * (3.14f / 180.0f), rtm_v3(0, 1, 0));
    c.cam_rz = rtm_rot_prepare(cam[5] * (3.14f / 180.0f), rtm_v3(0, 0, 1));
    c.ibl_x = rtm_rot_prepare(90.0f * (3.14f / 180.0f), rtm_v3(1, 0, 0));
    c.ibl_y = rtm_rot_prepare(90.0f * (3.14f / 180.0f), rtm_v3(0, 1, 0));
    rtm_f3 sun = rtm_v3(1, 1, 1);
    sun = rtm_rotate(F.env[0] * (3.14f / 180.0f), rtm_v3(1, 0, 0), sun);
    sun = rtm_rotate(F.env[1] * (3.14f / 180.0f), rtm_v3(0, 1, 0), sun);
    sun = rtm_rotate(F.env[2] * (3.14f / 180.0f), rtm_v3(0, 0, 1), sun);
    c.sun = sun;
    return c;
}

__global__ void make_const_kernel(FrameParams F, LaunchConst* __restrict__ out) {
    if (blockIdx.x == 0 && threadIdx.x == 0) *out = make_const(F);
}

inline size_t stack_lds_bytes(const DevScene& sc, int traversal, int block) {
    const int depth = traversal == TRAV_REF ? sc.ref_stack : (sc.nbrute > 0 ? 1 : 2 * std::max(sc.stack_lds, 1));
    const size_t lds = (size_t)depth * block * sizeof(int);
    return traversal == TRAV_FAST && sc.nbrute > 0 ? std::max(lds, (size_t)(block / 64) * BRUTE_WAVE_LDS) : lds;
}
inline size_t brute_lds_bytes(const DevScene& sc, int block, bool team) {
    if (!RT_SHADE_ROWS) team = true;
    const size_t shade = team ? (size_t)sc.nbox * 32 + (size_t)sc.ntri * 16 + (size_t)sc.nmat * (4 * kMatF)
                              : (size_t)sc.ntri * 32;
    return (size_t)(block / 64) * BRUTE_WAVE_LDS + (size_t)sc.nbrute * 48 + shade + (size_t)sc.ntri * 48 +
           (size_t)sc.ncslot * 32 + (sc.shell ? (size_t)kShellRows * 32 : 0);
}
inline size_t staged_scene_bytes(const DevScene& sc) {
    return (size_t)(kNodeF4 * sc.nnodes + 3 * sc.ntri) * sizeof(float4);
}

inline hipError_t setup_work_block(const FrameParams& f, unsigned int* d_work, hipStream_t stream,
                                   const LaunchConst** lconst) {
    static_assert(kConstOffset >= kGroups * kCounterStride && kConstOffset + sizeof(LaunchConst) <= kWorkBytes,
                  "work block layout");
    const hipError_t e = hipMemsetAsync(d_work, 0, (size_t)kGroups * kCounterStride, stream);
    if (e != hipSuccess) return e;
    LaunchConst* lc = reinterpret_cast<LaunchConst*>(reinterpret_cast<char*>(d_work) + kConstOffset);
    hipLaunchKernelGGL(make_const_kernel, dim3(1), dim3(64), 0, stream, f, lc);
    *lconst = lc;
    return hipGetLastError();
}

__device__ __forceinline__ rtm_f3 camera_dir(const LaunchConst& C, int W, int i) {
    const int pixelY = (i + 1) % W;
    const int pixelX = (i - pixelY) / W;
    const rtm_f3 pc = rtm_v3(fmaf((float)pixelY, C.pas, -0.5f), 0.0f, fmaf(-(float)pixelX, C.pas, 0.5f));
    rtm_f3 d = dev_normalize(rtm_sub(rtm_add(C.position, pc), C.focal));
    d = rtm_rot_apply(C.cam_rx, d);
    d = rtm_rot_apply(C.cam_ry, d);
    return rtm_rot_apply(C.cam_rz, d);
}

__global__ void ibl_sum_kernel(const uchar4* __restrict__ rgba, int w, int h, uint32_t* __restrict__ sum) {
    const int64_t n = (int64_t)(w + 1) * (h + 1);
    for (int64_t q = (int64_t)blockIdx.x * blockDim.x + threadIdx.x; q < n; q += (int64_t)gridDim.x * blockDim.x) {
        const int X = (int)(q % (w + 1)), Y = (int)(q / (w + 1));
        const int x0 = max(min(X - 1, w - 1), 0), x1 = min(X, w - 1);
        const int y0 = max(min(Y - 1, h - 1), 0), y1 = min(Y, h - 1);
        const uchar4 t00 = rgba[(int64_t)y0 * w + x0], t10 = rgba[(int64_t)y0 * w + x1];
        const uchar4 t01 = rgba[(int64_t)y1 * w + x0], t11 = rgba[(int64_t)y1 * w + x1];
        const uint32_t r = (uint32_t)t00.x + t10.x + t01.x + t11.x;
        const uint32_t g = (uint32_t)t00.y + t10.y + t01.y + t11.y;
// ... 809 lines not shown
```

ensem3a_openclraytracer_amd/csrc/rt_internal.h:

```cpp
#pragma once
#include <hip/hip_runtime.h>
#include <cstdint>

#include "rt_layout.h"
#include "rt_slices.h"

namespace rt {

constexpr int32_t kHostClusterAuto = 1;
constexpr int32_t kHostQuad = 2;
struct DevScene {
    const float4* nodes;
    int32_t nnodes;
    int32_t root_ref;
    const float4* wnodes;
    const float4* wleaves;
    int32_t wroot_ref;
    float wdq_omax;
    float root_box[6];
    const float* bvh9;
    int32_t nbvh9;
    int32_t ref_stack;
    const float4* tri_geo;
    const float4* tri_fast;
    const float4* tri_shade;
    const float4* tri_frame;
    int32_t ntri;
    const float* mat;
    int32_t nmat;
    uint32_t near_mask_hi;
    const uint32_t* ibl_sum;
    int32_t ibl_w, ibl_h;
    int32_t depth;
    int32_t stack_lds;
    int2* stack_ovf;
    const float4* brute;
    int32_t nbrute;
    uint32_t near_mask_lo;
    const float4* brute_box;
    int32_t nbox;
    float near_floor;
    const float4* brute_cbox;
    const float4* brute_crow;
    int32_t ncluster, ncslot, nsingle4;
    int32_t host_flags;
    int32_t nsingle;
    int32_t shell;
};

struct FrameParams {
    float cam[10];
    float env[5];
    int32_t width;
    int64_t npix;
    int32_t spp;
    int32_t max_bounce;
    int32_t row0, row_step;
    int64_t nloc;
    int32_t resume_min;
    int32_t team;
    int32_t walk_team;
    int32_t max_waves;
    int32_t handout;
    int32_t step;
    int32_t sun_skip;
    int32_t sun_any;
    int32_t wide;
    int32_t wdq;
    int32_t fixed_point;
    int32_t sun_cache;
    int32_t pass;
    int32_t pilot;
    int32_t pilot_chunk;
    int32_t pilot_levels;
    float4* pilot_state;
    uint32_t* pilot_cost;
    uint32_t* pilot_draws;
    int32_t spec;
    int32_t refill;
    float4* spec_log;
    int32_t spec_cap;
    int32_t slices;
    float4* slice_state;
    uint32_t* slice_ready;
    const uint32_t* pilot_order;
    int64_t log_pixel;
    float* log_buf;
    int32_t log_cap;
    int32_t* log_count;
};

struct RenderPending {
// ... 4 lines not shown
};
hipError_t launch_render(const DevScene& sc, const FrameParams& fp, int traversal, int block,
                         float* d_out, unsigned long long* d_counts, unsigned int* d_work, hipStream_t stream,
                         RenderPending* pend = nullptr);
hipError_t launch_render_finish(const DevScene& sc, int traversal, int block, float* d_out, unsigned int* d_work,
                                hipStream_t stream, RenderPending& pend);
hipError_t launch_accum(const DevScene& sc, const FrameParams& fp, float4* state, int base, int traversal, int block,
                        float* d_out, unsigned int* d_work, hipStream_t stream);
hipError_t launch_accum_listed(const DevScene& sc, const FrameParams& fp, float4* state, const uint32_t* list,
                               const uint32_t* count, int traversal, int block, float* d_out, unsigned int* d_work,
                               hipStream_t stream);
size_t select_scratch_words(int64_t n);
hipError_t launch_accum_mark(const float4* state, float4* mark, int64_t n, hipStream_t stream);
hipError_t launch_select_error(const float4* state, const float4* mark, uint8_t* flag, const FrameParams& fp,
                               float threshold, hipStream_t stream);
hipError_t launch_select_mask(const uint8_t* src, uint8_t* flag, const FrameParams& fp, hipStream_t stream);
hipError_t launch_select_compact(const uint8_t* flag, int64_t n, uint32_t* scratch, uint32_t* list, uint32_t* count,
                                 hipStream_t stream);
hipError_t launch_list_all(uint32_t* list, int64_t n, uint32_t* count, hipStream_t stream);
hipError_t launch_sample_map(const float4* state, int32_t* out, int64_t n, hipStream_t stream);
size_t launch_const_bytes();
hipError_t launch_accum_guides(const DevScene& sc, const FrameParams& fp, const float4* state, void* lconst,
                               float4* d_guides, hipStream_t stream);
size_t denoise_scratch_bytes(int64_t npix);
hipError_t launch_denoise(const float* d_rgb, const float4* d_guides, int64_t npix, int width, int passes, int nsq,
                          float sigma_c, float sigma_p, bool lds, float4* scratch, float* d_out,
                          hipStream_t stream);
hipError_t launch_accum_resolve(const float4* state, float* d_out, int64_t n, hipStream_t stream);
hipError_t launch_prep_frames(const DevScene& sc, float4* frame, hipStream_t stream);
hipError_t launch_ibl_sum(const uchar4* rgba, int w, int h, uint32_t* sum, hipStream_t stream);
hipError_t launch_gamma(const float* d_in, float* d_out, int64_t n, hipStream_t stream);
hipError_t launch_rgb8(const float* d_in, uint8_t* d_out, int64_t n, bool gamma, hipStream_t stream);
constexpr int kSpecTrails = 8;
constexpr int kSpecPick = 10;
constexpr int kSpecCapMax = 256;
constexpr int kWalkLanesPerCu = 4 * 4 * 64;
size_t spec_log_bytes(const FrameParams& fp, int cus);
hipError_t launch_spec(const DevScene& sc, const FrameParams& fp, int block, float* d_out, unsigned int* d_work,
                       hipStream_t stream);
constexpr int kRefillBrute = 4;
constexpr int kRefillMax = 64;
inline int brute_refill_launch(int option, int64_t nloc, int64_t lanes) {
    if (option >= 0) return option >= 2 ? (int)std::min<int64_t>(option, kRefillMax) : 0;
    return brute_auto_slices(nloc, lanes) ? kRefillBrute : 0;
}
struct KernelKey {
    int trav;
    int count;
    int log;
    int smem;
    int ovf;
    int resume;
    int step;
    int wide;
    int brute;
    int ts;
    int acc;
};
inline bool operator==(const KernelKey& a, const KernelKey& b) {
    return a.trav == b.trav && a.count == b.count && a.log == b.log && a.smem == b.smem && a.ovf == b.ovf &&
           a.resume == b.resume && a.step == b.step && a.wide == b.wide && a.brute == b.brute && a.ts == b.ts &&
           a.acc == b.acc;
}
KernelKey choose_kernel(const DevScene& sc, const FrameParams& fp, int traversal, bool count, bool log, int acc,
                        int block);
int64_t resident_blocks(const void* fn, int block, size_t lds, int max_waves, hipError_t* err);
struct QueryOptions {
    int engine;
    int grid_cap;
    int resume_min;
    int max_waves;
    int block;
};
hipError_t launch_query(const DevScene& sc, int traversal, int any, const float4* rays, float4* out, int64_t n,
                        const QueryOptions& q, unsigned int* counter, hipStream_t stream);
struct LaunchNote {
    KernelKey key;
    int team, walk_team, slices, refill;
    int64_t grid;
    size_t lds;
    int shell;
    int near;
    int quad;
};
void note_launch(const LaunchNote& n);
LaunchNote last_launch();
hipError_t launch_debug_math(int fn, const float* x, const float* y, float* out, int64_t n, hipStream_t stream);
hipError_t launch_debug_log(const DevScene& sc, const FrameParams& fp, int traversal, float* d_out,
                            unsigned int* d_work, hipStream_t stream);
hipError_t launch_debug_trace(const DevScene& sc, int traversal, const float* rays, float* out, int64_t n,
                              hipStream_t stream);
constexpr int kDebugFns = 9;
constexpr int debug_fn_in(int fn) {
    constexpr int w[kDebugFns] = {11, 5, 6, 13, 4, 24, 24, 12, 13};
    return fn >= 0 && fn < kDebugFns ? w[fn] : 0;
}
constexpr int debug_fn_out(int fn) {
    constexpr int w[kDebugFns] = {3, 3, 24, 3, 6, 2, 2, 1, 3};
    return fn >= 0 && fn < kDebugFns ? w[fn] : 0;
}
size_t debug_fn_scratch_bytes(int fn, int64_t n);
hipError_t launch_debug_fn(const DevScene& sc, int fn, const float* in, float* out, int64_t n, void* scratch,
                           hipStream_t stream);
hipError_t launch_debug_trace_clustered(const DevScene& sc, const float* rays, float* out, int64_t n, int32_t info[4],
                                        hipStream_t stream);

}
```

ensem3a_openclraytracer_amd/csrc/rt_kernels.hip:

```cpp
#include <mutex>
#include <vector>

#include "rt_device.h"

namespace rt {

namespace {

__device__ __forceinline__ void save_state(float4* __restrict__ st, int p, rtm_f3 acc, float kc, uint32_t seed0,
                                           uint32_t seed1, int tc, int s) {
    st[2 * (int64_t)p] = make_float4(acc.x, acc.y, acc.z, kc);
    st[2 * (int64_t)p + 1] =
        make_float4(__uint_as_float(seed0), __uint_as_float(seed1), __int_as_float(tc), __int_as_float(s));
}

[[maybe_unused]] constexpr int kAccAdd = 1;
constexpr int kAccListed = 2;
constexpr int kBruteSliced = 4;
constexpr int kBruteRefill = 8;
template <int TRAV, bool COUNT, bool LOG = false, bool SMEM = false, bool OVF = false, int BRUTE_ = 0, int ACC = 0>
#ifndef RT_RENDER_WAVES
#define RT_RENDER_WAVES 5
#endif
__global__ void __launch_bounds__(256) __attribute__((amdgpu_waves_per_eu(RT_RENDER_WAVES))) render_kernel(DevScene S, FrameParams F, float* __restrict__ out,
                                               unsigned long long* __restrict__ counts,
                                               unsigned int* __restrict__ work_counter,
                                               const LaunchConst* __restrict__ lconst) {
    constexpr int BRUTE = BRUTE_ & 3;
    constexpr bool SLICED = (BRUTE_ & kBruteSliced) != 0;
    static_assert(!SLICED || BRUTE == 1 || BRUTE == 3, "sample slices: the one-lane brute-force loops");
    constexpr bool kRefill = (BRUTE == 1 || BRUTE == 3) && ((BRUTE_ & kBruteRefill) != 0 || COUNT || LOG);
    static_assert(!(BRUTE_ & kBruteRefill) || BRUTE == 1 || BRUTE == 3, "refill threshold: the one-lane brute-force loops");
    extern __shared__ int lds_stack[];
    const int B = blockDim.x;
    int* stk = lds_stack + threadIdx.x;
    const LaneStack lst = lane_stack(S, lds_stack);
    Cnt c{};
    const float4* mtrec = nullptr;
    const float4* boxrec = nullptr;
    const float4* tshade = S.tri_shade;
    const float4* tframe = S.tri_frame;
    const float* tmat = S.mat;
    constexpr bool ROWS = RT_SHADE_ROWS && (BRUTE == 1 || BRUTE == 3);
    const float4* trow = nullptr;
    if (BRUTE) {
        float4* lr = reinterpret_cast<float4*>(reinterpret_cast<char*>(lds_stack) + (B / 64) * BRUTE_WAVE_LDS);
        float4* ls = lr + 3 * S.nbrute;
        if (BRUTE == 2) {
            for (int q = threadIdx.x; q < 2 * S.nbox; q += B) ls[q] = S.brute_box[q];
            boxrec = ls;
            ls += 2 * S.nbox;
        }
        float4* lf = ls + (ROWS ? 2 : 1) * S.ntri;
        float* lm = reinterpret_cast<float*>(lf + 3 * S.ntri);
        for (int q = threadIdx.x; q < 3 * S.nbrute; q += B) lr[q] = S.brute[4 * (q / 3) + 1 + q % 3];
        for (int q = threadIdx.x; q < 3 * S.ntri; q += B) lf[q] = S.tri_frame[q];
        if constexpr (ROWS) {
            for (int q = threadIdx.x; q < S.ntri; q += B) {
                const float4 sh = S.tri_shade[q];
                const float* m = S.mat + kMatF * __float_as_int(sh.w);
                ls[2 * q] = make_float4(sh.x, sh.y, sh.z, m[0]);
                ls[2 * q + 1] = make_float4(m[1], m[2], m[3], m[4]);
            }
            trow = ls;
        } else {
            for (int q = threadIdx.x; q < S.ntri; q += B) ls[q] = S.tri_shade[q];
            for (int q = threadIdx.x; q < kMatF * S.nmat; q += B) lm[q] = S.mat[q];
            tshade = ls;
            tmat = lm;
        }
        if (BRUTE == 3) {
            float4* lc = reinterpret_cast<float4*>(lm + (ROWS ? 0 : kMatF * S.nmat));
            for (int q = threadIdx.x; q < 2 * S.ncslot; q += B) lc[q] = S.brute_cbox[q];
            if (S.shell)
                for (int q = threadIdx.x; q < 2 * kShellRows; q += B) lc[S.shell + q] = S.brute_cbox[S.shell + kShellRowF4 + q];
            boxrec = lc;
        }
        __syncthreads();
        mtrec = lr;
        tframe = lf;
    }
    constexpr bool STAMPS = RT_CHAIN_STAMPS && BRUTE == 3 && !COUNT;
    [[maybe_unused]] char* const stamp_wl = reinterpret_cast<char*>(lds_stack) + (threadIdx.x >> 6) * BRUTE_WAVE_LDS;
    if constexpr (STAMPS) {
        if ((threadIdx.x & 63) == 0) {
            unsigned long long* st = reinterpret_cast<unsigned long long*>(stamp_wl + BRUTE_STAMP_OFF);
            for (int q = 0; q < kStampN; ++q) st[q] = 0;
            st[kStampN] = clock64();
        }
    }
    const LaunchConst& C = *lconst;
    const float4* nodes = S.nodes;
    const float4* tris = S.tri_fast;
    if (SMEM) {
        float4* ln = reinterpret_cast<float4*>(lds_stack + 2 * S.stack_lds * B);
        float4* lt = ln + kNodeF4 * S.nnodes;
        for (int q = threadIdx.x; q < kNodeF4 * S.nnodes; q += B)
            ln[(q % kNodeF4) * S.nnodes + q / kNodeF4] = S.nodes[q];
        for (int q = threadIdx.x; q < 3 * S.ntri; q += B) lt[q] = S.tri_fast[q];
        __syncthreads();
        nodes = ln;
        tris = lt;
    }
    const int W = F.width;
    const int imgSize = (int)F.npix;
    const float e3 = F.env[3], e4 = F.env[4];
    const int spp = F.spp, maxB = F.max_bounce;
    const unsigned int nloc = ACC == kAccListed ? (unsigned int)__builtin_amdgcn_readfirstlane((int)*F.pilot_cost)
                                                : (unsigned int)F.nloc;
    const int lane = threadIdx.x & 63;
    const int ts = BRUTE == 2 ? F.team : 1;
    const int team_lane0 = lane & ~(ts - 1);
    const bool team_leader = lane == team_lane0;
    const unsigned long long team_leaders = ts == 1 ? ~0ull : ts == 2 ? 0x5555555555555555ull
                                             : ts == 4 ? 0x1111111111111111ull : 0x0101010101010101ull;

    int phase = FETCH;
    PixelQueue pq;
    pq.per = (F.handout && F.pass != 2) ? (unsigned)(((ACC == kAccListed ? (int64_t)nloc : F.nloc) + kGroups - 1) / kGroups) : 0u;
    if constexpr (kRefill) pq.dry = F.refill > 1 ? (unsigned)min(F.refill, 64) << kQueueRefillShift : 0u;
    int p = 0, i = 0;
    bool logme = false;
    uint32_t seed0 = 0, seed1 = 0;
    rtm_f3 cd = rtm_v3(0, 0, 0);
    float kc = 1000.0f;
    int tc = -1;
    rtm_f3 so = rtm_v3(1, 1, 1);
    float k = 1000.0f;
    int tri = -1, j = 0;
    rtm_f3 Bo = rtm_v3(0, 0, 0), Bd = rtm_v3(0, 0, 0);
    rtm_f3 acc = rtm_v3(0, 0, 0);
    int s = 0;
    [[maybe_unused]] int plim = 0;
    auto slimit = [&]() __attribute__((always_inline)) { if constexpr (ACC == kAccListed) return plim; else return spp; };
    int cost = 0;
    int sun0 = -2;
    unsigned long long t_prev = 0;
    [[maybe_unused]] unsigned long long refill_ev = 0, refill_lanes = 0;
// ... 963 lines not shown
#endif

#if RT_CHAIN_STAMPS
namespace {
unsigned long long* chain_stamp_buffer() {
    static unsigned long long* p = [] {
        unsigned long long* q = nullptr;
        if (hipMalloc(&q, kStampN * sizeof(unsigned long long)) != hipSuccess) return (unsigned long long*)nullptr;
        if (hipMemset(q, 0, kStampN * sizeof(unsigned long long)) != hipSuccess) return (unsigned long long*)nullptr;
        return q;
    }();
    return p;
}
}
#ifndef RT_ACCUM_TU
extern "C" __attribute__((visibility("default"))) int rt_debug_chain_stamps(unsigned long long out[kStampN]) {
    unsigned long long* p = chain_stamp_buffer();
    if (!p || hipDeviceSynchronize() != hipSuccess) return 1;
    if (hipMemcpy(out, p, kStampN * sizeof(unsigned long long), hipMemcpyDeviceToHost) != hipSuccess) return 1;
    return hipMemset(p, 0, kStampN * sizeof(unsigned long long)) == hipSuccess ? 0 : 1;
}
#endif
#endif

namespace {
const void* kernel_fn(const KernelKey& k) {
    static const std::vector<KernelRow> table = [] {
        std::vector<KernelRow> t;
#ifndef RT_ACCUM_TU
        log_rows(t);
        head_rows<true>(t);
        head_rows<false>(t);
        engine_rows<true>(t);
#else
        head_rows<false>(t);
#endif
        engine_rows<false>(t);
        return t;
    }();
    for (const KernelRow& r : table)
        if (r.key == k) return r.fn;
    return nullptr;
}

hipError_t launch_pick(const DevScene& sc, const FrameParams& fp, KernelKey k, int block, float* d_out,
                       unsigned long long* d_counts, unsigned int* d_work, hipStream_t stream) {
    if (fp.nloc <= 0) return hipSuccess;
    const bool brute = k.brute != 0, product = !k.count && !k.log, listed = k.acc == kAccListed;
    size_t lds = (brute ? brute_lds_bytes(sc, block, true) : stack_lds_bytes(sc, k.trav, block)) +
                 (k.smem ? staged_scene_bytes(sc) : 0);
    hipError_t e = hipSuccess;
    auto resident = [&](int max_waves) { return resident_blocks(kernel_fn(k), block, lds, max_waves, &e); };
    if (brute && product && sc.ncluster > 0 && !((sc.host_flags & kHostClusterAuto) && fp.nloc < resident(0) * block)) k.brute = 3;
    const int64_t lanes = resident(fp.max_waves) * block;
    if (e != hipSuccess) return e;
    FrameParams f = fp;
    int bslices = 0;
    if (brute && !listed && fp.pass == 0 && fp.team <= 1 && fp.slice_state && fp.slice_ready &&
        sc.ntri + 2 < 65536 && fp.npix <= INT_MAX)
        bslices = brute_slice_launch(fp.slices, fp.nloc, lanes);
    if (!k.resume) f.slices = bslices;
    f.team = !brute ? 1 : bslices ? 1 : fp.team;
    if (f.team == 0) f.team = (!listed && fp.nloc * 4 <= lanes) ? 4 : 1;
    f.walk_team = 1;
    if (k.resume && k.step && !k.wide && !k.log) {
        f.walk_team = fp.walk_team ? fp.walk_team : listed ? 1 : auto_walk_team(fp.nloc, lanes);
        if (f.walk_team != 2 && f.walk_team != 4 && f.walk_team != 8) f.walk_team = 1;
    }
    f.refill = (brute && f.team <= 1) ? brute_refill_launch(fp.refill, fp.nloc, lanes) : 0;
    k.ts = f.walk_team;
    if (brute && f.team > 1) k.brute = 2;
    else if (brute) k.brute |= (bslices ? kBruteSliced : 0) | (product && f.refill > 1 ? kBruteRefill : 0);
    if (brute && f.team <= 1) lds = brute_lds_bytes(sc, block, false);
    const void* fn = kernel_fn(k);
    const int64_t need = (fp.nloc * f.team * f.walk_team + block - 1) / block;
    const int64_t grid = std::min(need, resident(fp.max_waves));
    if (e != hipSuccess) return e;
    if (bslices) e = hipMemsetAsync(f.slice_ready, 0, (size_t)fp.nloc * sizeof(uint32_t), stream);
    const LaunchConst* lc = nullptr;
    if (e == hipSuccess) e = setup_work_block(f, d_work, stream, &lc);
    if (e != hipSuccess) return e;
    const int shell = (k.brute & 3) == 3 && sc.shell != 0;
    note_launch({k, f.team, f.walk_team, f.slices, f.refill, grid, lds, shell, shell && sc.near_floor != 0.0f,
                 shell && (sc.host_flags & kHostQuad) != 0});
#if RT_CHAIN_STAMPS
    if (!d_counts) d_counts = chain_stamp_buffer();
#endif
    DevScene a0 = sc;
    void* args[] = {&a0, &f, &d_out, &d_counts, &d_work, &lc};
    return hipLaunchKernel(fn, dim3((unsigned)grid), dim3(block), args, lds, stream);
}

}

#ifndef RT_ACCUM_TU
hipError_t launch_debug_log(const DevScene& sc, const FrameParams& fp, int traversal, float* d_out,
                            unsigned int* d_work, hipStream_t stream) {
    return launch_pick(sc, fp, choose_kernel(sc, fp, traversal, false, true, 0, 64), 64, d_out, nullptr, d_work, stream);
}

constexpr int kCostBins = 256;

__global__ void pilot_chunk_kernel(const uint32_t* __restrict__ cost, int64_t nfull, int chunk,
                                   uint32_t* __restrict__ ccost) {
    for (int64_t c = (int64_t)blockIdx.x * blockDim.x + threadIdx.x; c < nfull; c += (int64_t)gridDim.x * blockDim.x) {
        uint32_t t = 0;
        for (int k = 0; k < chunk; ++k) t += cost[c * chunk + k];
        ccost[c] = t;
    }
}

__device__ __forceinline__ uint32_t cost_bin(uint32_t v, uint32_t scale, uint32_t maxbin) {
    return min(maxbin, (uint32_t)(((uint64_t)v * scale) >> 16));
}

constexpr int kSortSeg = kCostBins;

__global__ void pilot_seg_hist_kernel(const uint32_t* __restrict__ ccost, int64_t n, int64_t nseg, uint32_t scale,
                                      uint32_t maxbin, uint32_t* __restrict__ seghist) {
    __shared__ uint32_t h[kCostBins];
    const int64_t seg = blockIdx.x;
    h[threadIdx.x] = 0;
    __syncthreads();
    const int64_t q = seg * kSortSeg + threadIdx.x;
    if (q < n) atomicAdd(&h[cost_bin(ccost[q], scale, maxbin)], 1u);
    __syncthreads();
    seghist[threadIdx.x * nseg + seg] = h[threadIdx.x];
}

__global__ void pilot_seg_scan_kernel(uint32_t* __restrict__ seghist, int64_t nseg, uint32_t* __restrict__ total) {
    __shared__ uint32_t t[kCostBins];
    uint32_t* row = seghist + (int64_t)blockIdx.x * nseg;
    const int i0 = threadIdx.x;
    uint32_t carry = 0;
    for (int64_t base = 0; base < nseg; base += kCostBins) {
        const int64_t i = base + i0;
        const uint32_t v = i < nseg ? row[i] : 0u;
        t[i0] = v;
        __syncthreads();
        for (int off = 1; off < kCostBins; off <<= 1) {
            const uint32_t a = i0 >= off ? t[i0 - off] : 0u;
            __syncthreads();
            t[i0] += a;
            __syncthreads();
        }
        if (i < nseg) row[i] = carry + t[i0] - v;
        carry += t[kCostBins - 1];
        __syncthreads();
    }
    if (i0 == 0) total[blockIdx.x] = carry;
}

__global__ void pilot_scan_kernel(const uint32_t* __restrict__ hist, uint32_t* __restrict__ offs) {
    __shared__ uint32_t t[kCostBins];
    const int b = threadIdx.x;
    t[b] = hist[b];
    __syncthreads();
    uint32_t above = 0;
    for (int c = b + 1; c < kCostBins; ++c) above += t[c];
    offs[b] = above;
}

__global__ void pilot_seg_scatter_kernel(const uint32_t* __restrict__ ccost, int64_t n, int64_t nseg, uint32_t scale,
                                         uint32_t maxbin, const uint32_t* __restrict__ seghist,
                                         const uint32_t* __restrict__ offs, uint32_t* __restrict__ corder) {
    __shared__ uint32_t bins[kSortSeg];
    const int64_t seg = blockIdx.x;
// ... 344 lines not shown
```

ensem3a_openclraytracer_amd/csrc/rt_layout.h:

```cpp
#pragma once
#include <cstddef>
#include <cstdint>

namespace rt {

constexpr int kStackLds = 20;
constexpr int kStackLdsWide = 11;
#ifndef RT_WIDE_WAVES
#define RT_WIDE_WAVES 7
#endif
constexpr int kWideWaves = RT_WIDE_WAVES;
constexpr int kNodeF4 = 4;
constexpr int kMaxLanesPerCu = 2048;
#ifndef RT_BOX_GROUP
#define RT_BOX_GROUP 4
#endif
constexpr int kBoxGroup = RT_BOX_GROUP;
constexpr int kClusterShift = 3;
constexpr int kClusterSlots = 1 << kClusterShift;
constexpr double kClusterKappa = 1.9;
constexpr double kClusterGain = 0.75;
constexpr int kClusterLockNum = 4;
constexpr int kShellRows = 7;
constexpr int kShellRowF4 = 5;
constexpr int kShellRecF = 20 + 8 * kShellRows;
constexpr int kShellMinFaces = 3;
constexpr float kQuadBand = 0x1p-8f;
constexpr float kQuadGraze = 0x1p-6f;
constexpr float kQuadDirMax = 2.0f;
constexpr double kQuadSafety = 8.0;
constexpr double kQuadSlack = 0x1p-20;
constexpr double kQuadRatio = 4.0;
constexpr double kQuadKappa = 4.0;
constexpr int kQuadExp = 24;
constexpr float kNearFloor = 0.0001f * (1.0f - 0x1p-12f);
constexpr double kNearKappa = 256.0;
constexpr int kNearExp = 40;
#ifndef RT_BRUTE_MAX_DEFAULT
#define RT_BRUTE_MAX_DEFAULT 64
#endif
constexpr int kMatF = 8;
constexpr size_t kWideMinBytes = 16u << 20;

constexpr int kGroups = 8;
constexpr int kCounterStride = 64;
constexpr int kTeamOffset = 512;
constexpr int kConstOffset = 1024;
constexpr int kWorkBytes = 2048;
constexpr int kChunkShift = 10;

}
```

ensem3a_openclraytracer_amd/csrc/scene_pack.cpp:

```cpp
#include "scene_pack.h"

#include <algorithm>
#include <array>
#include <cmath>
#include <cstdarg>
#include <cstdio>
#include <cstring>
#include <atomic>
#include <functional>
#include <map>
#include <mutex>
#include <new>
#include <stdexcept>
#include <string>
#include <system_error>
#include <thread>
#include <vector>

#include "../../include/rt_api.h"
#include "../../include/rt_debug.h"
#include "../../include/rt_scene.h"
#include "bvh_sah.h"

using rt::HostScene;
// ... 751 lines not shown
    hs.brute_shell.clear();
    hs.nshell = 0;
    hs.nrest = 0;
    hs.brute_near.clear();
    hs.shell_floor = 0.0f;
    hs.shell_mask = 0;
    hs.nquad = 0;
    if ((int64_t)leaves.size() <= (int64_t)brute_max) {
        std::vector<int32_t> by_rank(leaves.size());
        for (int32_t n : leaves) by_rank[rank[T[n]]] = n;
        hs.brute.assign(16 * by_rank.size(), 0.0f);
        for (size_t q = 0; q < by_rank.size(); ++q) {
            const float* nd = bvh9 + 9 * (int64_t)by_rank[q];
            const int32_t t = T[by_rank[q]];
            const float* g = hs.tri_geo.data() + 12 * t;
            float* r = hs.brute.data() + 16 * q;
            r[0] = nd[2]; r[1] = nd[3]; r[2] = nd[4]; r[3] = nd[5];
            r[4] = nd[6]; r[5] = nd[7]; r[6] = g[0]; r[7] = g[1];
            r[8] = g[2]; r[9] = g[4]; r[10] = g[5]; r[11] = g[6];
            r[12] = g[8]; r[13] = g[9]; r[14] = g[10]; r[15] = as_f32(t);
        }
        hs.nbrute = (int32_t)by_rank.size();
        std::vector<std::array<int32_t, 2>> groups;
        {
            std::map<std::array<uint32_t, 6>, size_t> open;
            for (size_t q = 0; q < by_rank.size(); ++q) {
                const float* r = hs.brute.data() + 16 * q;
                std::array<uint32_t, 6> key;
                for (int k = 0; k < 6; ++k) std::memcpy(&key[k], r + k, 4);
                auto it = open.find(key);
                if (it != open.end()) {
                    groups[it->second][1] = (int32_t)q;
                    open.erase(it);
                } else {
                    open[key] = groups.size();
                    groups.push_back({(int32_t)q, -1});
                }
            }
        }
        hs.nbox = (int32_t)groups.size();
        const size_t ng = (groups.size() + rt::kBoxGroup - 1) / rt::kBoxGroup * rt::kBoxGroup;
        hs.brute_box.assign(8 * ng, 0.0f);
        for (size_t g = 0; g < ng; ++g) {
            float* b = hs.brute_box.data() + 8 * g;
            if (g < groups.size()) {
                const float* r = hs.brute.data() + 16 * groups[g][0];
                b[0] = r[0]; b[1] = r[3];
                b[2] = r[1]; b[3] = r[4];
                b[4] = r[2]; b[5] = r[5];
                b[6] = as_f32(groups[g][0]); b[7] = as_f32(groups[g][1]);
            } else {
                pad_box(b);
            }
        }
        hs.brute_near.assign((size_t)hs.nbox, 0);
        for (int32_t g = 0; g < hs.nbox; ++g) hs.brute_near[g] = near_safe(hs, hs.brute_box.data() + 8 * (size_t)g);
        build_clusters(hs, cluster);
        build_shell(hs, shell, quad);
    }
    if (layout == RT_BVH_SAH && leaves.size() > 1) {
        std::vector<float> lb(6 * leaves.size());
        std::vector<int32_t> ids(leaves.size());
        for (size_t q = 0; q < leaves.size(); ++q) {
            const float* nd = bvh9 + 9 * (int64_t)leaves[q];
            for (int k = 0; k < 6; ++k) lb[6 * q + k] = nd[2 + k];
            ids[q] = T[leaves[q]];
        }
        rt::SahTree st;
        rt::sah_build(lb.data(), ids.data(), (int64_t)leaves.size(), st);
        emit_bvh(hs, st.L.data(), st.R.data(), st.leaf.data(), st.box.data(), (int64_t)st.L.size());
        return true;
    }
    std::vector<float> box(6 * nn);
    for (int64_t i = 0; i < nn; ++i)
        for (int k = 0; k < 6; ++k) box[6 * i + k] = bvh9[9 * i + 2 + k];
    emit_bvh(hs, L.data(), R.data(), T.data(), box.data(), nn);
    return true;
}

}

namespace rt {

void pack_checked(HostScene& hs, const float* bvh9, int64_t nb, int64_t ntri, int layout, int brute_max, int cluster,
                  int shell, int quad, std::string& why) {
    hs.fast_ok = (ntri > 0) ? pack_fast(hs, bvh9, nb, ntri, layout, brute_max, cluster, shell, quad, why) : true;
    if (hs.fast_ok && ntri > 0) {
        double m1 = 0.0, m2 = 0.0;
        for (int64_t t = 0; t < ntri; ++t) {
            const float* g = hs.tri_geo.data() + 12 * t;
            const double l1 = std::sqrt((double)g[4] * g[4] + (double)g[5] * g[5] + (double)g[6] * g[6]);
            const double l2 = std::sqrt((double)g[8] * g[8] + (double)g[9] * g[9] + (double)g[10] * g[10]);
            if (std::isfinite(l1)) m1 = std::max(m1, l1);
            if (std::isfinite(l2)) m2 = std::max(m2, l2);
        }
        if (!(m1 * m2 <= std::ldexp(1.0, 120))) {
            hs.fast_ok = false;
            why = "triangle edges beyond 2^60 (the FAST reciprocal needs |e1 . (d x e2)| <= 2^126)";
        }
    }
    if (ntri == 0) {
        hs.nnodes = 0; hs.root_ref = 0; hs.depth = 1; hs.nodes.clear();
        hs.nwnodes = 0; hs.wroot_ref = 0; hs.wdepth = 1; hs.wnodes.clear(); hs.wleaves.clear();
        hs.brute.clear(); hs.brute_box.clear(); hs.nbrute = 0; hs.nbox = 0;
    }
    if (!hs.fast_ok) { hs.brute.clear(); hs.brute_box.clear(); hs.nbrute = 0; hs.nbox = 0; }
    if (hs.nbrute == 0) { hs.brute_cbox.clear(); hs.brute_crow.clear(); hs.ncluster = 0; hs.nsingle = 0; hs.brute_near.clear(); }
    if (hs.ncluster == 0) { hs.brute_shell.clear(); hs.nshell = 0; hs.nrest = 0; hs.shell_floor = 0.0f; hs.shell_mask = 0; hs.nquad = 0; }
    if (!hs.fast_ok || hs.wdepth > 64) { hs.wnodes.clear(); hs.wleaves.clear(); hs.nwnodes = 0; hs.wdepth = 1; }
    if (hs.fast_ok && hs.depth > 64) {
        hs.fast_ok = false;
        why = "tree deeper than 64 levels";
    }
    if (hs.nodes.empty()) hs.nodes.assign(4 * rt::kNodeF4, 0.0f);
    if (hs.brute.empty()) hs.brute.assign(16, 0.0f);
    if (hs.brute_box.empty()) {
        hs.brute_box.assign(8 * rt::kBoxGroup, 0.0f);
        for (int g = 0; g < rt::kBoxGroup; ++g) pad_box(hs.brute_box.data() + 8 * g);
    }
}

namespace {

int scene_prepare_(HostScene& hs, const float* vp, int64_t nvp, const float* vn, int64_t nvn, const int32_t* face,
                   int64_t nface, const float* mat, int64_t nmat, const float* bvh9, int64_t nbvh, int layout,
                   int brute_max, int cluster, int shell, int quad, std::string& msg, std::string& why) {
    if (nvp < 0 || nvp % 3 || nvn < 0 || nvn % 3 || nface < 0 || nface % 10 || nmat <= 0 || nmat % 6 || nbvh < 0 ||
        nbvh % 9)
        return fail(msg, RT_ERR_ARG,
                       "bad array sizes (V_p %lld, V_n %lld, faceData %lld, materialData %lld, BVH %lld)",
                       (long long)nvp, (long long)nvn, (long long)nface, (long long)nmat, (long long)nbvh);
    if ((nface && (!vp || !vn || !face)) || !mat || (nbvh && !bvh9))
        return fail(msg, RT_ERR_ARG, "null array");
    const int64_t T = nface / 10, NV = nvp / 3, NN = nvn / 3, M = nmat / 6, NB = nbvh / 9;
    if (T > 0x3fffffff || NB > 0x7fffffff) return fail(msg, RT_ERR_ARG, "scene too large");
    if (T > 0 && NB == 0) return fail(msg, RT_ERR_SCENE, "triangles given without a BVH");
    for (int64_t m = 0; m < M; ++m) {
        const float tf = mat[6 * m];
        if (!(tf > -1.0f && tf < 4.0f))
            return fail(msg, RT_ERR_SCENE, "material %lld has type %g; the kernel defines types 0..3", (long long)m,
                           (double)tf);
    }
    hs.ntri = (int32_t)T;
    hs.nmat = (int32_t)M;
    hs.nbvh9 = (int32_t)NB;
    hs.mat.assign((size_t)rt::kMatF * M, 0.0f);
    for (int64_t m = 0; m < M; ++m) {
        for (int k = 0; k < 6; ++k) hs.mat[(size_t)rt::kMatF * m + k] = mat[6 * m + k];
        for (int k = 1; k < 4; ++k) hs.colors_finite = hs.colors_finite && std::isfinite(mat[6 * m + k]);
        hs.has_glass = hs.has_glass || (int)mat[6 * m] == 3;
    }
    if (bvh9) hs.bvh9.assign(bvh9, bvh9 + nbvh);
    hs.tri_geo.assign((size_t)T * 12, 0.0f);
    hs.tri_shade.assign((size_t)T * 4, 0.0f);
    for (int64_t t = 0; t < T; ++t) {
        const int32_t* f = face + 10 * t;
        if (f[0] < 0 || f[0] >= M)
            return fail(msg, RT_ERR_ARG, "triangle %lld: material %d out of range [0,%lld)", (long long)t, f[0],
                           (long long)M);
        for (int j = 7; j < 10; ++j)
            if (f[j] < 0 || f[j] >= NV)
                return fail(msg, RT_ERR_ARG, "triangle %lld: position index %d out of range", (long long)t, f[j]);
        if (f[4] < 0 || f[4] >= NN)
            return fail(msg, RT_ERR_ARG, "triangle %lld: normal index %d out of range", (long long)t, f[4]);
        const float* a = vp + 3 * (int64_t)f[7];
        const float* b = vp + 3 * (int64_t)f[8];
// ... 121 lines not shown
        return RT_ERR_ARG;
    }
    if (cluster < -1 || cluster > 1) {
        g_check_error = "brute_cluster must be -1 (auto), 0 (off) or 1 (force)";
        return RT_ERR_ARG;
    }
    if (!info || slot_cap < 0 || row_cap < 0 || (slot_cap > 0 && !slots) || (row_cap > 0 && !rows)) {
        g_check_error = "null info, or a capacity without an array";
        return RT_ERR_ARG;
    }
    const int rc = rt::scene_prepare(hs, vp, nvp, vn, nvn, face, nface, mat, nmat, bvh9, nbvh, layout,
                                     RT_BRUTE_MAX_DEFAULT, cluster, -1, -1, msg, why);
    g_check_error = rc != RT_OK ? msg : hs.fast_ok ? std::string() : "FAST traversal unavailable (" + why + ")";
    if (rc != RT_OK) return rc;
    info[0] = hs.ncluster;
    info[1] = hs.nsingle;
    info[2] = (int64_t)hs.brute_cbox.size();
    info[3] = (int64_t)hs.brute_crow.size();
    const int64_t ns = std::min<int64_t>(slot_cap, info[2]), nr = std::min<int64_t>(row_cap, info[3]);
    if (ns > 0) std::memcpy(slots, hs.brute_cbox.data(), (size_t)ns * sizeof(float));
    if (nr > 0) std::memcpy(rows, hs.brute_crow.data(), (size_t)nr * sizeof(float));
    return RT_OK;
}

extern "C" int rt_debug_brute_shell(const float* vp, int64_t nvp, const float* vn, int64_t nvn, const int32_t* face,
                                    int64_t nface, const float* mat, int64_t nmat, const float* bvh9, int64_t nbvh,
                                    int layout, int cluster, int shell, float* rec, int64_t cap, int64_t info[3]) {
    HostScene hs;
    std::string msg, why;
    if (layout != RT_BVH_REFERENCE && layout != RT_BVH_SAH) {
        g_check_error = "layout must be RT_BVH_REFERENCE or RT_BVH_SAH";
        return RT_ERR_ARG;
    }
    if (cluster < -1 || cluster > 1 || shell < -1 || shell > 1) {
        g_check_error = "brute_cluster and brute_shell must be -1 (auto), 0 (off) or 1 (force)";
        return RT_ERR_ARG;
    }
    if (!info || cap < 0 || (cap > 0 && !rec)) {
        g_check_error = "null info, or a capacity without an array";
        return RT_ERR_ARG;
    }
    const int rc = rt::scene_prepare(hs, vp, nvp, vn, nvn, face, nface, mat, nmat, bvh9, nbvh, layout,
                                     RT_BRUTE_MAX_DEFAULT, cluster, shell, -1, msg, why);
    g_check_error = rc != RT_OK ? msg : hs.fast_ok ? std::string() : "FAST traversal unavailable (" + why + ")";
    if (rc != RT_OK) return rc;
    info[0] = hs.nshell;
    info[1] = hs.nrest;
    info[2] = (int64_t)hs.brute_shell.size();
    const int64_t n = std::min<int64_t>(cap, info[2]);
    if (n > 0) std::memcpy(rec, hs.brute_shell.data(), (size_t)n * sizeof(float));
    return RT_OK;
}

extern "C" int rt_debug_brute_near(const float* vp, int64_t nvp, const float* vn, int64_t nvn, const int32_t* face,
                                   int64_t nface, const float* mat, int64_t nmat, const float* bvh9, int64_t nbvh,
                                   int layout, int cluster, int shell, int32_t* flags, int64_t cap, float* floor,
                                   int64_t info[2]) {
    HostScene hs;
    std::string msg, why;
    if (layout != RT_BVH_REFERENCE && layout != RT_BVH_SAH) {
        g_check_error = "layout must be RT_BVH_REFERENCE or RT_BVH_SAH";
        return RT_ERR_ARG;
    }
    if (cluster < -1 || cluster > 1 || shell < -1 || shell > 1) {
        g_check_error = "brute_cluster and brute_shell must be -1 (auto), 0 (off) or 1 (force)";
        return RT_ERR_ARG;
    }
    if (!info || !floor || cap < 0 || (cap > 0 && !flags)) {
        g_check_error = "null info or floor, or a capacity without an array";
        return RT_ERR_ARG;
    }
    const int rc = rt::scene_prepare(hs, vp, nvp, vn, nvn, face, nface, mat, nmat, bvh9, nbvh, layout,
                                     RT_BRUTE_MAX_DEFAULT, cluster, shell, -1, msg, why);
    g_check_error = rc != RT_OK ? msg : hs.fast_ok ? std::string() : "FAST traversal unavailable (" + why + ")";
    if (rc != RT_OK) return rc;
    info[0] = (int64_t)hs.brute_near.size();
    info[1] = hs.nshell;
    *floor = hs.shell_floor;
    const int64_t n = std::min<int64_t>(cap, info[0]);
    for (int64_t g = 0; g < n; ++g) flags[g] = hs.brute_near[(size_t)g];
    return RT_OK;
}

extern "C" int rt_debug_brute_quad(const float* vp, int64_t nvp, const float* vn, int64_t nvn, const int32_t* face,
                                   int64_t nface, const float* mat, int64_t nmat, const float* bvh9, int64_t nbvh,
                                   int layout, int cluster, int shell, int quad, int32_t flags[6], float lines[24],
                                   int32_t words[18], float recs[108], float guard[3], int64_t info[2]) {
    HostScene hs;
    std::string msg, why;
    if (layout != RT_BVH_REFERENCE && layout != RT_BVH_SAH) {
        g_check_error = "layout must be RT_BVH_REFERENCE or RT_BVH_SAH";
        return RT_ERR_ARG;
    }
    if (cluster < -1 || cluster > 1 || shell < -1 || shell > 1) {
        g_check_error = "brute_cluster and brute_shell must be -1 (auto), 0 (off) or 1 (force)";
        return RT_ERR_ARG;
    }
    if (quad < -1 || quad > 1) {
        g_check_error = "brute_quad must be -1 (auto), 0 (off) or 1 (auto)";
        return RT_ERR_ARG;
    }
    if (!info || !flags || !lines || !words || !recs || !guard) {
        g_check_error = "null info, flags, lines, words, recs or guard";
        return RT_ERR_ARG;
    }
    const int rc = rt::scene_prepare(hs, vp, nvp, vn, nvn, face, nface, mat, nmat, bvh9, nbvh, layout,
                                     RT_BRUTE_MAX_DEFAULT, cluster, shell, quad, msg, why);
    g_check_error = rc != RT_OK ? msg : hs.fast_ok ? std::string() : "FAST traversal unavailable (" + why + ")";
    if (rc != RT_OK) return rc;
    info[0] = hs.nshell;
    info[1] = hs.nquad;
    guard[0] = rt::kQuadBand; guard[1] = rt::kQuadGraze; guard[2] = rt::kQuadDirMax;
    for (int f = 0; f < 6; ++f) {
        flags[f] = 0;
        for (int k = 0; k < 4; ++k) lines[4 * f + k] = 0.0f;
        for (int k = 0; k < 3; ++k) words[3 * f + k] = -1;
        for (int k = 0; k < 18; ++k) recs[18 * f + k] = 0.0f;
        if (hs.nshell == 0) continue;
        const float* row = hs.brute_shell.data() + 4 * rt::kShellRowF4 + 8 * f;
        std::memcpy(lines + 4 * f, row, 16);
        std::memcpy(words + 3 * f, row + 4, 12);
        std::memcpy(flags + f, row + 7, 4);
        const uint32_t both = (uint32_t)words[3 * f];
        for (int j = 0; j < 2; ++j) {
            const uint32_t q = j ? both >> 16 : both & 0xffffu;
            if (both != ~0u && q != 0xffffu && (int32_t)q < hs.nbrute)
                std::memcpy(recs + 18 * f + 9 * j, hs.brute.data() + 16 * (size_t)q + 6, 9 * sizeof(float));
        }
    }
    return RT_OK;
}
```

ensem3a_openclraytracer_amd/csrc/scene_pack.h:

```cpp
#pragma once
#include <cstdint>
#include <string>
#include <vector>

#include "rt_layout.h"

namespace rt {

struct HostScene {
    std::vector<float> nodes;
    std::vector<float> wnodes;
    std::vector<float> wleaves;
    int32_t nwnodes = 0, wroot_ref = 0, wdepth = 1;
    float wdq_omax = 0.0f;
    std::vector<float> bvh9;
    std::vector<float> tri_geo;
    std::vector<float> tri_fast;
    std::vector<float> tri_shade;
    std::vector<float> mat;
    std::vector<float> brute;
    std::vector<float> brute_box;
    int32_t nbrute = 0;
    int32_t nbox = 0;
    std::vector<float> brute_cbox;
    std::vector<float> brute_crow;
    int32_t ncluster = 0, nsingle = 0;
    std::vector<float> brute_shell;
    int32_t nshell = 0, nrest = 0;
    int32_t nquad = 0;
    std::vector<uint8_t> brute_near;
    float shell_floor = 0.0f;
    uint64_t shell_mask = 0;
    int32_t nnodes = 0, root_ref = 0, ntri = 0, nmat = 0, nbvh9 = 0, depth = 1;
    float root_box[6] = {0, 0, 0, 0, 0, 0};
    bool fast_ok = false;
    bool colors_finite = true;
    bool has_glass = false;
};


int scene_prepare(HostScene& hs, const float* vp, int64_t nvp, const float* vn, int64_t nvn, const int32_t* face,
                  int64_t nface, const float* mat, int64_t nmat, const float* bvh9, int64_t nbvh, int layout,
                  int brute_max, int cluster, int shell, int quad, std::string& msg, std::string& why);

void pack_checked(HostScene& hs, const float* bvh9, int64_t nb, int64_t ntri, int layout, int brute_max, int cluster,
                  int shell, int quad, std::string& why);

}
```

include/rt_debug.h:

```cpp
#ifndef RT_DEBUG_H
#define RT_DEBUG_H

#include <stdint.h>
#include "rt_api.h"


#ifdef __cplusplus
extern "C" {
#endif

int rt_debug_math(rt_ctx* ctx, int fn, const float* x, const float* y, float* out, int64_t n);

int rt_debug_trace(rt_ctx* ctx, int traversal, const float* rays, float* out, int64_t n);

int rt_debug_trace_clustered(rt_ctx* ctx, const float* rays, float* out, int64_t n, int32_t info[4]);

enum {
    RT_FN_CAMERA = 0, RT_FN_SUN = 1, RT_FN_HEMI = 2, RT_FN_GGX = 3, RT_FN_IBL = 4, RT_FN_MT_REF = 5,
    RT_FN_MT_FAST = 6, RT_FN_BOX_REF = 7, RT_FN_BOX_FAST = 8, RT_FN_COUNT = 9
};
int rt_debug_fn(rt_ctx* ctx, int fn, const float* in, float* out, int64_t n);

int rt_debug_pixel_log(rt_ctx* ctx, int traversal, const float cam[10], const float env[5], int64_t npix, int spp,
                       int max_bounce, int64_t pixel, float* log, int cap, int* n_events, float out3[3]);

int rt_debug_wave_counts(rt_ctx* ctx, const float cam[10], const float env[5], int64_t npix, int spp,
                         int max_bounce, uint64_t out[9]);

int rt_debug_scene_info(rt_ctx* ctx, int64_t out[8]);

int rt_debug_timings(rt_ctx* ctx, double out[4]);

int rt_debug_quantise_axis(float p, const float* lo, const float* hi, int n, float gap, uint8_t* qlo, uint8_t* qhi);

int rt_debug_brute_layout(const float* V_p, int64_t n_vp, const float* V_n, int64_t n_vn, const int32_t* faceData,
                          int64_t n_face, const float* materialData, int64_t n_mat, const float* bvh, int64_t n_bvh,
                          int layout, float* boxes, int64_t cap, int64_t info[3]);

int rt_debug_brute_clusters(const float* V_p, int64_t n_vp, const float* V_n, int64_t n_vn, const int32_t* faceData,
                            int64_t n_face, const float* materialData, int64_t n_mat, const float* bvh, int64_t n_bvh,
                            int layout, int cluster, float* slots, int64_t slot_cap, float* rows, int64_t row_cap,
                            int64_t info[4]);

int rt_debug_brute_shell(const float* V_p, int64_t n_vp, const float* V_n, int64_t n_vn, const int32_t* faceData,
                         int64_t n_face, const float* materialData, int64_t n_mat, const float* bvh, int64_t n_bvh,
                         int layout, int cluster, int shell, float* rec, int64_t cap, int64_t info[3]);

int rt_debug_brute_near(const float* V_p, int64_t n_vp, const float* V_n, int64_t n_vn, const int32_t* faceData,
                        int64_t n_face, const float* materialData, int64_t n_mat, const float* bvh, int64_t n_bvh,
                        int layout, int cluster, int shell, int32_t* flags, int64_t cap, float* floor, int64_t info[2]);

int rt_debug_brute_quad(const float* V_p, int64_t n_vp, const float* V_n, int64_t n_vn, const int32_t* faceData,
                        int64_t n_face, const float* materialData, int64_t n_mat, const float* bvh, int64_t n_bvh,
                        int layout, int cluster, int shell, int quad, int32_t flags[6], float lines[24],
                        int32_t words[18], float recs[108], float guard[3], int64_t info[2]);

int rt_debug_brute_slices(int64_t nloc, int64_t lanes, int spp, int option, int accum_base, int32_t out[3]);

int rt_debug_last_slices(void);

int rt_debug_last_launch(int32_t out[20]);

int rt_debug_brute_refill(int64_t nloc, int64_t lanes, int option, int32_t* out);

int rt_debug_last_refill(int64_t out[3]);

#ifdef __cplusplus
}
#endif
#endif
```

Measured before the change: 12380 Msamples/s.

## Repack LDS triangle records and test first shell candidate directly per lane

Changes the LDS Möller–Trumbore record layout so vertex and edges pack into contiguous float4s, with the triangle id at float index 9. Adds a 'direct' shell mode, on by default when a shell exists: each lane intersects its first candidate triangle in place instead of pushing it through the ring and batch path. Only the second candidate goes through the ring. This is meant to cut ring traffic, LDS syncs and batch rounds, at the cost of more divergent per-lane work and added complexity in the packed shell word.

```diff
diff --git a/ensem3a_openclraytracer_amd/_native.py b/ensem3a_openclraytracer_amd/_native.py
--- a/ensem3a_openclraytracer_amd/_native.py
+++ b/ensem3a_openclraytracer_amd/_native.py
@@ -34,6 +34,7 @@
     "rt_bvh_build", "rt_device_count", "rt_debug_math", "rt_debug_fn", "rt_debug_trace", "rt_debug_trace_clustered", "rt_debug_scene_info", "rt_debug_pixel_log",
     "rt_debug_wave_counts", "rt_debug_quantise_axis", "rt_debug_timings", "rt_debug_brute_layout",
     "rt_debug_brute_clusters", "rt_debug_brute_shell", "rt_debug_brute_near", "rt_debug_brute_quad",
+    "rt_debug_brute_direct", "rt_debug_last_direct", "rt_debug_shell_word",
     "rt_debug_brute_slices",
     "rt_debug_last_slices",
     "rt_debug_brute_refill", "rt_debug_last_refill", "rt_debug_last_launch",
@@ -542,6 +543,11 @@
         self._check(lib().rt_debug_trace_clustered(self.handle, r.ctypes.data, out.ctypes.data, len(r), info.ctypes.data))
         return out[:, 0].copy(), out[:, 1].copy().view(np.int32), info
 
+    def shell_word(self) -> int:
+        fn = lib().rt_debug_shell_word
+        fn.restype, fn.argtypes = _i32, [_c_p]
+        return int(fn(self.handle))
+
     def debug_pixel_log(self, traversal, cam, env, npix, spp, max_bounce, pixel, cap=4096):
         c, e = f32(cam), f32(env)
         log = np.zeros((cap, 16), np.float32)
@@ -697,6 +703,29 @@
                 words=words.view(np.uint32).reshape(6, 3), recs=recs.reshape(6, 2, 3, 3), guard=guard, nfaces=int(info[0]), nsplit=int(info[1]))
 
 
+SHELL_DIRECT = 1 << 16
+
+
+def brute_direct(V_p, V_n, faceData, materialData, bvh, cluster: int = -1, shell: int = -1, direct: int = -1,
+                 layout: int = RT_BVH_SAH):
+    vp, vn, face, mat, b = f32(V_p), f32(V_n), i32(faceData), f32(materialData), f32(bvh)
+    H = host_lib()
+    fn = H.rt_debug_brute_direct
+    fn.restype, fn.argtypes = _i32, [_c_p, _i64, _c_p, _i64, _c_p, _i64, _c_p, _i64, _c_p, _i64, _i32, _i32, _i32, _i32, _c_p]
+    info = np.zeros(3, np.int64)
+    st = fn(ptr(vp), vp.size, ptr(vn), vn.size, ptr(face), face.size, ptr(mat), mat.size, ptr(b), b.size, int(layout),
+            int(cluster), int(shell), int(direct), info.ctypes.data)
+    if st != 0:
+        raise NativeError(st, H.rt_scene_last_error().decode(errors="replace"))
+    return int(info[0]), bool(info[1]), int(info[2])
+
+
+def last_direct() -> bool:
+    fn = lib().rt_debug_last_direct
+    fn.restype, fn.argtypes = _i32, []
+    return bool(fn())
+
+
 def brute_slices(nloc: int, lanes: int, spp: int, option: int = -1, accum_base: int = -1):
     out = np.zeros(3, np.int32)
     st = lib().rt_debug_brute_slices(int(nloc), int(lanes), int(spp), int(option), int(accum_base), out.ctypes.data)
diff --git a/ensem3a_openclraytracer_amd/csrc/rt_api.hip b/ensem3a_openclraytracer_amd/csrc/rt_api.hip
--- a/ensem3a_openclraytracer_amd/csrc/rt_api.hip
+++ b/ensem3a_openclraytracer_amd/csrc/rt_api.hip
@@ -103,6 +103,7 @@
     int brute_cluster = -1;
     int brute_shell = -1;
     int brute_near = -1;
+    int brute_direct = -1;
     int brute_quad = -1;
     int resume_min = -1;
     int team = 0;
@@ -276,7 +277,8 @@
     s.ncluster = ctx->hs.ncluster;
     s.ncslot = (int32_t)(ctx->hs.brute_cbox.size() / 8);
     s.nsingle4 = s.ncslot - rt::kClusterSlots * s.ncluster;
-    s.host_flags = (ctx->brute_cluster < 0 ? rt::kHostClusterAuto : 0) | (ctx->hs.nquad > 0 ? rt::kHostQuad : 0);
+    s.host_flags = (ctx->brute_cluster < 0 ? rt::kHostClusterAuto : 0) | (ctx->hs.nquad > 0 ? rt::kHostQuad : 0) |
+                   (ctx->hs.nshell > 0 && ctx->brute_direct != 0 ? rt::kHostDirect : 0);
     s.nsingle = ctx->hs.nsingle;
     s.shell = ctx->hs.nshell > 0 ? 2 * s.ncslot : 0;
     s.near_floor = s.shell && ctx->brute_near != 0 ? ctx->hs.shell_floor : 0.0f;
@@ -365,6 +367,7 @@
     std::string why;
     rt::pack_checked(hs, hs.bvh9.data(), hs.nbvh9, hs.ntri, ctx->bvh_layout, ctx->brute_max, ctx->brute_cluster,
                      ctx->brute_shell, ctx->brute_quad, why);
+    rt::shell_direct(hs, ctx->brute_direct);
     for (auto& d : ctx->devs) {
         const int st = upload_fast(ctx, d, hs);
         if (st) return st;
@@ -413,6 +416,7 @@
         {"traversal", &rt_ctx::traversal, range(RT_TRAVERSAL_FAST, RT_TRAVERSAL_REF), "traversal must be 0 (fast) or 1 (ref)", invalidate},
         {"brute_near", &rt_ctx::brute_near, range(-1, 1), "brute_near must be -1 (auto), 0 (off) or 1 (auto)", none},
         {"brute_quad", &rt_ctx::brute_quad, range(-1, 1), "brute_quad must be -1 (auto), 0 (off) or 1 (auto)", repack},
+        {"brute_direct", &rt_ctx::brute_direct, range(-1, 1), "brute_direct must be -1 (auto), 0 (off) or 1 (auto)", repack},
         {"bvh", &rt_ctx::bvh_layout, range(RT_BVH_REFERENCE, RT_BVH_SAH), "bvh must be 0 (reference tree) or 1 (sah)", repack},
         {"brute_cluster", &rt_ctx::brute_cluster, range(-1, 1), "brute_cluster must be -1 (auto), 0 (off) or 1 (force)", repack},
         {"brute_shell", &rt_ctx::brute_shell, range(-1, 1), "brute_shell must be -1 (auto), 0 (off) or 1 (force)", repack},
@@ -525,6 +529,7 @@
     const int rc = rt::scene_prepare(hs, vp, nvp, vn, nvn, face, nface, mat, nmat, bvh9, nbvh, ctx->bvh_layout,
                                      ctx->brute_max, ctx->brute_cluster, ctx->brute_shell, ctx->brute_quad, msg, why);
     if (rc != RT_OK) return set_err(ctx, rc, "%s", msg.c_str());
+    rt::shell_direct(hs, ctx->brute_direct);
     invalidate_accum(ctx);
     const auto t1 = std::chrono::steady_clock::now();
     for (auto& d : ctx->devs) {
@@ -1682,6 +1687,15 @@
 
 int rt_debug_last_slices(void) { return rt::last_launch().slices; }
 
+int rt_debug_last_direct(void) { return rt::last_launch().direct; }
+
+int rt_debug_shell_word(rt_ctx* ctx) {
+    if (!ctx || !ctx->have_scene || ctx->hs.nshell <= 0 || ctx->hs.brute_shell.size() < 8) return 0;
+    int32_t w;
+    std::memcpy(&w, &ctx->hs.brute_shell[7], sizeof w);
+    return w;
+}
+
 int rt_debug_last_launch(int32_t out[20]) {
     if (!out) return RT_ERR_ARG;
     const rt::LaunchNote n = rt::last_launch();
diff --git a/ensem3a_openclraytracer_amd/csrc/rt_debug_fn.hip b/ensem3a_openclraytracer_amd/csrc/rt_debug_fn.hip
--- a/ensem3a_openclraytracer_amd/csrc/rt_debug_fn.hip
+++ b/ensem3a_openclraytracer_amd/csrc/rt_debug_fn.hip
@@ -123,11 +123,11 @@
 
 __global__ void __launch_bounds__(256) debug_trace_clustered_kernel(DevScene S, const float* __restrict__ rays,
                                                                     float* __restrict__ out, int64_t n) {
-    extern __shared__ int lds_stack[];
+    extern __shared__ __attribute__((aligned(16))) int lds_stack[];
     const int B = blockDim.x;
     float4* lr = reinterpret_cast<float4*>(reinterpret_cast<char*>(lds_stack) + (B / 64) * BRUTE_WAVE_LDS);
     float4* lc = lr + 3 * S.nbrute;
-    for (int q = threadIdx.x; q < 3 * S.nbrute; q += B) lr[q] = S.brute[4 * (q / 3) + 1 + q % 3];
+    stage_mt_records(lr, S.brute, S.nbrute);
     for (int q = threadIdx.x; q < 2 * S.ncslot; q += B) lc[q] = S.brute_cbox[q];
     if (S.shell)
         for (int q = threadIdx.x; q < 2 * kShellRows; q += B) lc[S.shell + q] = S.brute_cbox[S.shell + kShellRowF4 + q];
diff --git a/ensem3a_openclraytracer_amd/csrc/rt_device.h b/ensem3a_openclraytracer_amd/csrc/rt_device.h
--- a/ensem3a_openclraytracer_amd/csrc/rt_device.h
+++ b/ensem3a_openclraytracer_amd/csrc/rt_device.h
@@ -407,12 +407,27 @@
     return __float_as_uint(sure ? (sg >= 0.0f ? wd.y : wd.z) : wd.x);
 }
 
+#ifndef RT_WIDE_REC
+#define RT_WIDE_REC 1
+#endif
+static_assert(BRUTE_WAVE_LDS % 16 == 0 && BRUTE_INV_OFF % 16 == 0 && BRUTE_STAMP_OFF % 16 == 0, "16-byte LDS tables");
+__device__ __forceinline__ void stage_mt_records(float4* lr, const float4* brute, int nbrute) {
+    for (int q = threadIdx.x; q < nbrute; q += blockDim.x) {
+        const float4 g1 = brute[4 * q + 1], g2 = brute[4 * q + 2], g3 = brute[4 * q + 3];
+        if (!RT_WIDE_REC) { lr[3 * q] = g1; lr[3 * q + 1] = g2; lr[3 * q + 2] = g3; continue; }
+        lr[3 * q] = make_float4(g1.z, g1.w, g2.x, g2.y);
+        lr[3 * q + 1] = make_float4(g2.z, g2.w, g3.x, g3.y);
+        lr[3 * q + 2] = make_float4(g3.z, g3.w, 0.0f, 0.0f);
+    }
+}
+
 template <int N> struct IntC { static constexpr int value = N; };
 static_assert(kBoxGroup == 1 || kBoxGroup == 2 || kBoxGroup == 4 || kBoxGroup == 8, "the lock-step tail is cut into powers of two");
 
-template <bool COUNT, bool CLU = false>
+template <bool COUNT, bool CLU = false, bool LREC_ = CLU>
 __device__ Hit trace_brute_compact(const DevScene& S, rtm_f3 o, rtm_f3 d, char* wl, const float4* mtrec,
                                    unsigned mtstride, Cnt& c, int ts = 1, const float4* boxrec = nullptr) {
+    constexpr bool LREC = LREC_ && RT_WIDE_REC;
     const unsigned lane = threadIdx.x & 63;
     const unsigned sub = lane & (unsigned)(ts - 1), tl = lane - sub;
     if (COUNT && sub == 0) c.rays++;
@@ -431,6 +446,23 @@
     float bk = 1000.0f;
     unsigned head = 0, tail = 0;
     [[maybe_unused]] int sec = kStampShell;
+    [[maybe_unused]] auto mt_pair = [&](const rtm_f3 ro, const rtm_f3 rd, unsigned q, float& k) __attribute__((always_inline)) {
+        const float4* rq = mtrec + mtstride * q;
+        const float4 r1 = rq[0], r2 = rq[1];
+        const float r3 = reinterpret_cast<const float*>(rq)[8];
+        const rtm_f3 a = rtm_v3(r1.x, r1.y, r1.z), e1 = rtm_v3(r1.w, r2.x, r2.y), e2 = rtm_v3(r2.z, r2.w, r3);
+        const rtm_f3 h = rtm_cross(rd, e2);
+        const float det = rtm_dot(e1, h);
+        const float f = mt_recip(det);
+        const rtm_f3 sv = rtm_sub(ro, a);
+        const float u = f * rtm_dot(sv, h);
+        const rtm_f3 qv = rtm_cross(sv, e1);
+        const float v = f * rtm_dot(rd, qv);
+        k = f * rtm_dot(e2, qv);
+        const bool parallel = det > -0.0000001f && det < 0.0000001f;
+        return !parallel && !(u < 0.0f || u > 1.0f) && !(v < 0.0f || u + v > 1.0f) &&
+               (k > 0.0000001f) && k > 0.0001f && k < 1000.0f;
+    };
     auto run_batch = [&](int n) __attribute__((always_inline)) {
         if constexpr (CLU && !COUNT) chain_stamp(wl, sec);
         if (myrank < n) {
@@ -438,21 +470,26 @@
             const unsigned ow = e >> 16, q = e & 0xffffu;
             const rtm_f3 ro = rtm_v3(ray[ow], ray[64 + ow], ray[128 + ow]);
             const rtm_f3 rd = rtm_v3(ray[192 + ow], ray[256 + ow], ray[320 + ow]);
-            const float4* rq = mtrec + mtstride * q;
-            const float4 r1 = rq[0], r2 = rq[1], r3 = rq[2];
-            const rtm_f3 a = rtm_v3(r1.z, r1.w, r2.x), e1 = rtm_v3(r2.y, r2.z, r2.w), e2 = rtm_v3(r3.x, r3.y, r3.z);
-            const rtm_f3 h = rtm_cross(rd, e2);
-            const float det = rtm_dot(e1, h);
-            const float f = mt_recip(det);
-            const rtm_f3 sv = rtm_sub(ro, a);
-            const float u = f * rtm_dot(sv, h);
-            const rtm_f3 qv = rtm_cross(sv, e1);
-            const float v = f * rtm_dot(rd, qv);
-            const float k = f * rtm_dot(e2, qv);
-            const bool parallel = det > -0.0000001f && det < 0.0000001f;
-            const bool hit = !parallel && !(u < 0.0f || u > 1.0f) && !(v < 0.0f || u + v > 1.0f) &&
-                             (k > 0.0000001f) && k > 0.0001f && k < 1000.0f;
-            if (hit) atomicMin(&bestk[ow], ((unsigned long long)__float_as_uint(k) << 32) | q);
+            if constexpr (LREC) {
+                float k;
+                if (mt_pair(ro, rd, q, k)) atomicMin(&bestk[ow], ((unsigned long long)__float_as_uint(k) << 32) | q);
+            } else {
+                const float4* rq = mtrec + mtstride * q;
+                const float4 r1 = rq[0], r2 = rq[1], r3 = rq[2];
+                const rtm_f3 a = rtm_v3(r1.z, r1.w, r2.x), e1 = rtm_v3(r2.y, r2.z, r2.w), e2 = rtm_v3(r3.x, r3.y, r3.z);
+                const rtm_f3 h = rtm_cross(rd, e2);
+                const float det = rtm_dot(e1, h);
+                const float f = mt_recip(det);
+                const rtm_f3 sv = rtm_sub(ro, a);
+                const float u = f * rtm_dot(sv, h);
+                const rtm_f3 qv = rtm_cross(sv, e1);
+                const float v = f * rtm_dot(rd, qv);
+                const float k = f * rtm_dot(e2, qv);
+                const bool parallel = det > -0.0000001f && det < 0.0000001f;
+                const bool hit = !parallel && !(u < 0.0f || u > 1.0f) && !(v < 0.0f || u + v > 1.0f) &&
+                                 (k > 0.0000001f) && k > 0.0001f && k < 1000.0f;
+                if (hit) atomicMin(&bestk[ow], ((unsigned long long)__float_as_uint(k) << 32) | q);
+            }
         }
         head += n;
         wave_lds_sync();
@@ -530,7 +567,8 @@
         if (S.shell) {
             const ConstF4 sh{cb.p + 4 * S.shell};
             const float4 h0 = sgpr4(sh[0]), h1 = sgpr4(sh[1]), fx = sgpr4(sh[2]), fy = sgpr4(sh[3]), fz = sgpr4(sh[4]);
-            const int nquad = __float_as_int(h1.w) >> 8;
+            const int nquad = (__float_as_int(h1.w) >> 8) & 0xff;
+            [[maybe_unused]] const bool direct = (__float_as_int(h1.w) & kShellDirect) != 0;
             const float cull = bk * CULL_MARGIN, nearf = S.near_floor;
             const float x0 = (h0.x - o.x) * ix, x1 = (h0.y - o.x) * ix;
             const float y0 = (h0.z - o.y) * iy, y1 = (h0.w - o.y) * iy;
@@ -571,7 +609,23 @@
                 }
                 const bool p1 = pk != ~0u, p2 = pk < 0xffff0000u;
                 const unsigned long long m1 = __ballot(p1);
-                if (m1 != 0) {
+                if (LREC && !COUNT && direct && m1 != 0) {
+                    const unsigned q1 = p1 ? (pk & 0xffffu) : 0u;
+                    float k1;
+                    const bool hit1 = mt_pair(o, d, q1, k1) && p1;
+                    bestk[lane] = hit1 ? ((unsigned long long)__float_as_uint(k1) << 32) | q1 : nokey;
+                    bk = hit1 ? k1 : bk;
+                    const unsigned long long m2 = __ballot(p2);
+                    if (m2 != 0) {
+                        ring[p2 ? (lane_prefix(m2, tail) & (BRUTE_RING - 1)) : BRUTE_RING + lane] = (tl << 16) | (pk >> 16);
+                        tail += (unsigned)__popcll(m2);
+                    }
+                    wave_lds_sync();
+                    if ((int)(tail - head) >= nact) {
+                        do run_batch(nact); while ((int)(tail - head) >= nact);
+                        bk = __uint_as_float((unsigned)(bestk[tl] >> 32));
+                    }
+                } else if (m1 != 0) {
                     const unsigned long long m2 = __ballot(p2);
                     const unsigned n1 = (unsigned)__popcll(m1);
                     if (COUNT && p1) c.tris += p2 ? 2 : 1;
@@ -709,7 +763,8 @@
     Hit best{1000.0f, -1};
     if (key != nokey) {
         best.k = __uint_as_float((unsigned)(key >> 32));
-        best.tri = __float_as_int(mtrec[mtstride * (unsigned)(key & 0xffffffffu) + 2].w);
+        const float4* rq = mtrec + mtstride * (unsigned)(key & 0xffffffffu);
+        best.tri = __float_as_int(LREC ? reinterpret_cast<const float*>(rq)[9] : rq[2].w);
     }
     if constexpr (CLU && !COUNT) chain_stamp(wl, kStampTail);
     return best;
@@ -721,7 +776,7 @@
                                      int ts = 1, const float4* boxrec = nullptr) {
     if (TRAV == TRAV_REF) return trace_ref<COUNT>(S, o, d, stk, B, c);
     if (S.nbrute > 0)
-        return trace_brute_compact<COUNT, CLU>(S, o, d, reinterpret_cast<char*>(stk - threadIdx.x) +
+        return trace_brute_compact<COUNT, CLU, BLDS>(S, o, d, reinterpret_cast<char*>(stk - threadIdx.x) +
                                                         (threadIdx.x >> 6) * BRUTE_WAVE_LDS,
                                           BLDS ? mtrec : S.brute + 1, BLDS ? 3u : 4u, c, BLDS ? ts : 1, boxrec);
     return trace_fast<COUNT, SOA, OVF>(S, nodes, tris, o, d, st, c);
diff --git a/ensem3a_openclraytracer_amd/csrc/rt_internal.h b/ensem3a_openclraytracer_amd/csrc/rt_internal.h
--- a/ensem3a_openclraytracer_amd/csrc/rt_internal.h
+++ b/ensem3a_openclraytracer_amd/csrc/rt_internal.h
@@ -8,6 +8,7 @@
 namespace rt {
 
 constexpr int32_t kHostClusterAuto = 1;
+constexpr int32_t kHostDirect = 4;
 constexpr int32_t kHostQuad = 2;
 struct DevScene {
     const float4* nodes;
@@ -178,6 +179,7 @@
     int shell;
     int near;
     int quad;
+    int direct;
 };
 void note_launch(const LaunchNote& n);
 LaunchNote last_launch();
diff --git a/ensem3a_openclraytracer_amd/csrc/rt_kernels.hip b/ensem3a_openclraytracer_amd/csrc/rt_kernels.hip
--- a/ensem3a_openclraytracer_amd/csrc/rt_kernels.hip
+++ b/ensem3a_openclraytracer_amd/csrc/rt_kernels.hip
@@ -31,7 +31,7 @@
     static_assert(!SLICED || BRUTE == 1 || BRUTE == 3, "sample slices: the one-lane brute-force loops");
     constexpr bool kRefill = (BRUTE == 1 || BRUTE == 3) && ((BRUTE_ & kBruteRefill) != 0 || COUNT || LOG);
     static_assert(!(BRUTE_ & kBruteRefill) || BRUTE == 1 || BRUTE == 3, "refill threshold: the one-lane brute-force loops");
-    extern __shared__ int lds_stack[];
+    extern __shared__ __attribute__((aligned(16))) int lds_stack[];
     const int B = blockDim.x;
     int* stk = lds_stack + threadIdx.x;
     const LaneStack lst = lane_stack(S, lds_stack);
@@ -53,7 +53,7 @@
         }
         float4* lf = ls + (ROWS ? 2 : 1) * S.ntri;
         float* lm = reinterpret_cast<float*>(lf + 3 * S.ntri);
-        for (int q = threadIdx.x; q < 3 * S.nbrute; q += B) lr[q] = S.brute[4 * (q / 3) + 1 + q % 3];
+        stage_mt_records(lr, S.brute, S.nbrute);
         for (int q = threadIdx.x; q < 3 * S.ntri; q += B) lf[q] = S.tri_frame[q];
         if constexpr (ROWS) {
             for (int q = threadIdx.x; q < S.ntri; q += B) {
@@ -1183,7 +1183,7 @@
     if (e != hipSuccess) return e;
     const int shell = (k.brute & 3) == 3 && sc.shell != 0;
     note_launch({k, f.team, f.walk_team, f.slices, f.refill, grid, lds, shell, shell && sc.near_floor != 0.0f,
-                 shell && (sc.host_flags & kHostQuad) != 0});
+                 shell && (sc.host_flags & kHostQuad) != 0, shell && (sc.host_flags & kHostDirect) != 0});
 #if RT_CHAIN_STAMPS
     if (!d_counts) d_counts = chain_stamp_buffer();
 #endif
diff --git a/ensem3a_openclraytracer_amd/csrc/rt_layout.h b/ensem3a_openclraytracer_amd/csrc/rt_layout.h
--- a/ensem3a_openclraytracer_amd/csrc/rt_layout.h
+++ b/ensem3a_openclraytracer_amd/csrc/rt_layout.h
@@ -25,6 +25,7 @@
 constexpr int kShellRowF4 = 5;
 constexpr int kShellRecF = 20 + 8 * kShellRows;
 constexpr int kShellMinFaces = 3;
+constexpr int32_t kShellDirect = 1 << 16;
 constexpr float kQuadBand = 0x1p-8f;
 constexpr float kQuadGraze = 0x1p-6f;
 constexpr float kQuadDirMax = 2.0f;
diff --git a/ensem3a_openclraytracer_amd/csrc/scene_pack.cpp b/ensem3a_openclraytracer_amd/csrc/scene_pack.cpp
--- a/ensem3a_openclraytracer_amd/csrc/scene_pack.cpp
+++ b/ensem3a_openclraytracer_amd/csrc/scene_pack.cpp
@@ -857,6 +857,13 @@
 
 namespace rt {
 
+bool shell_direct(HostScene& hs, int direct) {
+    if (hs.nshell <= 0 || hs.brute_shell.size() < (size_t)rt::kShellRecF) return false;
+    const int32_t w = as_i32(hs.brute_shell[7]);
+    hs.brute_shell[7] = as_f32(direct != 0 ? (w | rt::kShellDirect) : (w & ~rt::kShellDirect));
+    return direct != 0;
+}
+
 void pack_checked(HostScene& hs, const float* bvh9, int64_t nb, int64_t ntri, int layout, int brute_max, int cluster,
                   int shell, int quad, std::string& why) {
     hs.fast_ok = (ntri > 0) ? pack_fast(hs, bvh9, nb, ntri, layout, brute_max, cluster, shell, quad, why) : true;
@@ -1144,6 +1151,37 @@
     return RT_OK;
 }
 
+extern "C" int rt_debug_brute_direct(const float* vp, int64_t nvp, const float* vn, int64_t nvn, const int32_t* face,
+                                     int64_t nface, const float* mat, int64_t nmat, const float* bvh9, int64_t nbvh,
+                                     int layout, int cluster, int shell, int direct, int64_t info[3]) {
+    HostScene hs;
+    std::string msg, why;
+    if (layout != RT_BVH_REFERENCE && layout != RT_BVH_SAH) {
+        g_check_error = "layout must be RT_BVH_REFERENCE or RT_BVH_SAH";
+        return RT_ERR_ARG;
+    }
+    if (cluster < -1 || cluster > 1 || shell < -1 || shell > 1) {
+        g_check_error = "brute_cluster and brute_shell must be -1 (auto), 0 (off) or 1 (force)";
+        return RT_ERR_ARG;
+    }
+    if (direct < -1 || direct > 1) {
+        g_check_error = "brute_direct must be -1 (auto), 0 (off) or 1 (auto)";
+        return RT_ERR_ARG;
+    }
+    if (!info) {
+        g_check_error = "null info";
+        return RT_ERR_ARG;
+    }
+    const int rc = rt::scene_prepare(hs, vp, nvp, vn, nvn, face, nface, mat, nmat, bvh9, nbvh, layout,
+                                     RT_BRUTE_MAX_DEFAULT, cluster, shell, -1, msg, why);
+    g_check_error = rc != RT_OK ? msg : hs.fast_ok ? std::string() : "FAST traversal unavailable (" + why + ")";
+    if (rc != RT_OK) return rc;
+    info[1] = rt::shell_direct(hs, direct) ? 1 : 0;
+    info[0] = hs.nshell;
+    info[2] = hs.nshell > 0 ? (int64_t)as_i32(hs.brute_shell[7]) : 0;
+    return RT_OK;
+}
+
 extern "C" int rt_debug_brute_quad(const float* vp, int64_t nvp, const float* vn, int64_t nvn, const int32_t* face,
                                    int64_t nface, const float* mat, int64_t nmat, const float* bvh9, int64_t nbvh,
                                    int layout, int cluster, int shell, int quad, int32_t flags[6], float lines[24],
diff --git a/ensem3a_openclraytracer_amd/csrc/scene_pack.h b/ensem3a_openclraytracer_amd/csrc/scene_pack.h
--- a/ensem3a_openclraytracer_amd/csrc/scene_pack.h
+++ b/ensem3a_openclraytracer_amd/csrc/scene_pack.h
@@ -46,4 +46,6 @@
 void pack_checked(HostScene& hs, const float* bvh9, int64_t nb, int64_t ntri, int layout, int brute_max, int cluster,
                   int shell, int quad, std::string& why);
 
+bool shell_direct(HostScene& hs, int direct);
+
 }
diff --git a/include/rt_debug.h b/include/rt_debug.h
--- a/include/rt_debug.h
+++ b/include/rt_debug.h
@@ -55,6 +55,14 @@
                         int layout, int cluster, int shell, int quad, int32_t flags[6], float lines[24],
                         int32_t words[18], float recs[108], float guard[3], int64_t info[2]);
 
+int rt_debug_brute_direct(const float* V_p, int64_t n_vp, const float* V_n, int64_t n_vn, const int32_t* faceData,
+                          int64_t n_face, const float* materialData, int64_t n_mat, const float* bvh, int64_t n_bvh,
+                          int layout, int cluster, int shell, int direct, int64_t info[3]);
+
+int rt_debug_last_direct(void);
+
+int rt_debug_shell_word(rt_ctx* ctx);
+
 int rt_debug_brute_slices(int64_t nloc, int64_t lanes, int spp, int option, int accum_base, int32_t out[3]);
 
 int rt_debug_last_slices(void);
```

After: 12640 Msamples/s (median of 6 runs). 2.1% higher.
